# t-0hmura/pdb2reaction

Measured on AMD Instinct MI355X. Metric: path_opt_string_iterations_per_s, higher is better.
Workload: dtype bf16x3-split

## Files before the change

pdb2reaction_amd/csrc/gemm_bench.hip:

```cpp
#include <hip/hip_runtime.h>
#include <algorithm>
#include <cmath>
#include <cstdio>
#include <cstdlib>
#include <cstring>
#include <vector>
#include "umx_gemm_pl.h"
#include "umx_gemm_q.h"
using namespace umx;
#define CK(x) do { hipError_t e = (x); if (e != hipSuccess) { printf("HIP error %s at %s:%d\n", hipGetErrorString(e), __FILE__, __LINE__); exit(1); } } while (0)

template <class F> float timeit(F f, int reps = 5) {
  hipEvent_t a, b; CK(hipEventCreate(&a)); CK(hipEventCreate(&b));
  f(); CK(hipDeviceSynchronize());
  CK(hipEventRecord(a)); for (int i = 0; i < reps; ++i) f(); CK(hipEventRecord(b)); CK(hipEventSynchronize(b));
  float ms; CK(hipEventElapsedTime(&ms, a, b)); return ms / reps;
}

template <int P>
__global__ void k_split(const float* __restrict__ src, long rows, long ld, int K, unsigned short* __restrict__ dst) {
  const long i = (long)blockIdx.x * blockDim.x + threadIdx.x;
  if (i >= rows * K) return;
  const long r = i / K; const int k = (int)(i % K);
  float x = src[r * ld + k];
  for (int q = 0; q < P; ++q) { const __bf16 h = (__bf16)x; dst[r * K * P + (k / 32) * 32 * P + q * 32 + (k % 32)] = __builtin_bit_cast(unsigned short, h); x -= (float)h; }
}

template <int P>
__global__ void k_split_q(const float* __restrict__ src, long rows, long ld, int K, unsigned char* __restrict__ dst) {
  const long i = (long)blockIdx.x * blockDim.x + threadIdx.x;
  if (i >= rows * K) return;
  const long r = i / K; const int k = (int)(i % K);
  float x = src[r * ld + k];
  unsigned short* d = reinterpret_cast<unsigned short*>(dst + ((r / 4) * (K / 16) + k / 16) * (128 * P) + (r % 4) * (32 * P) + (k % 16) * 2);
  for (int q = 0; q < P; ++q) { const __bf16 hh = (__bf16)x; d[q * 16] = __builtin_bit_cast(unsigned short, hh); x -= (float)hh; }
}

template <int PQ>
__global__ void k_split_q_f16(const float* __restrict__ src, long rows, long ld, int K, unsigned char* __restrict__ dst) {
  const long i = (long)blockIdx.x * blockDim.x + threadIdx.x;
  if (i >= rows * K) return;
  const long r = i / K; const int k = (int)(i % K);
  float x = src[r * ld + k];
  unsigned short* d = reinterpret_cast<unsigned short*>(dst + ((r / 4) * (K / 16) + k / 16) * (128 * PQ) + (r % 4) * (32 * PQ) + (k % 16) * 2);
  for (int q = 0; q < PQ; ++q) { const _Float16 hq = (_Float16)x; d[16 * q] = __builtin_bit_cast(unsigned short, hq); x -= (float)hq; }
}

constexpr int Q8_SHIFT = 20;
constexpr int Q8_SHIFT1 = 10;
template <int WEIGHT>
__global__ void k_split_o8(const float* __restrict__ src, long rows, long ld, int K, unsigned char* __restrict__ dst) {
  const long i = (long)blockIdx.x * blockDim.x + threadIdx.x;
  if (i >= rows * K) return;
  const long r = i / K; const int k = (int)(i % K);
  const float x = src[r * ld + k];
  const _Float16 h0 = (_Float16)x; const _Float16 h1 = (_Float16)(x - (float)h0);
  const float r2 = (x - (float)h0) - (float)h1;
  const float xc = fminf(fmaxf(x, -57344.f), 57344.f), l1 = (float)h1 * (float)(1 << Q8_SHIFT1);
  const int pk = WEIGHT ? __builtin_amdgcn_cvt_pk_bf8_f32(xc, l1, 0, false) : __builtin_amdgcn_cvt_pk_bf8_f32(l1, r2 * (float)(1 << Q8_SHIFT), 0, false);
  unsigned char* d = dst + (r * (K / 64) + k / 64) * 128 + (k % 64);
  d[0] = (unsigned char)(pk & 0xff); d[64] = (unsigned char)((pk >> 8) & 0xff);
}


__global__ void k_copy_qf(const float* __restrict__ src, long rows, long ld, int K, unsigned char* __restrict__ dst) {
  const long i = (long)blockIdx.x * blockDim.x + threadIdx.x;
  if (i >= rows * K) return;
  const long r = i / K; const int k = (int)(i % K);
  *reinterpret_cast<float*>(dst + ((r / 4) * (K / 16) + k / 16) * 256 + (r % 4) * 64 + (k % 16) * 4) = src[r * ld + k];
}
typedef float f32x4_t __attribute__((ext_vector_type(4)));
typedef unsigned int u32x4_t __attribute__((ext_vector_type(4)));
#ifndef QF_TRUNC
#define QF_TRUNC 0
#endif
__device__ __forceinline__ void split3_pair(float x0, float x1, unsigned int& p0, unsigned int& p1, unsigned int& p2) {
#if QF_TRUNC
  const unsigned int u0 = __builtin_bit_cast(unsigned int, x0), u1 = __builtin_bit_cast(unsigned int, x1);
  p0 = __builtin_amdgcn_perm(u1, u0, 0x07060302u);
  const float r0 = x0 - __builtin_bit_cast(float, u0 & 0xffff0000u), r1 = x1 - __builtin_bit_cast(float, u1 & 0xffff0000u);
  const unsigned int v0 = __builtin_bit_cast(unsigned int, r0), v1 = __builtin_bit_cast(unsigned int, r1);
  p1 = __builtin_amdgcn_perm(v1, v0, 0x07060302u);
  const float s0 = r0 - __builtin_bit_cast(float, v0 & 0xffff0000u), s1 = r1 - __builtin_bit_cast(float, v1 & 0xffff0000u);
  p2 = __builtin_amdgcn_perm(__builtin_bit_cast(unsigned int, s1), __builtin_bit_cast(unsigned int, s0), 0x07060302u);
#else
  typedef float f32x2_t __attribute__((ext_vector_type(2)));
  typedef __bf16 bf16x2_t __attribute__((ext_vector_type(2)));
  p0 = __builtin_bit_cast(unsigned int, __builtin_convertvector(f32x2_t{x0, x1}, bf16x2_t));
  const float r0 = x0 - __builtin_bit_cast(float, p0 << 16), r1 = x1 - __builtin_bit_cast(float, p0 & 0xffff0000u);
  p1 = __builtin_bit_cast(unsigned int, __builtin_convertvector(f32x2_t{r0, r1}, bf16x2_t));
  const float s0 = r0 - __builtin_bit_cast(float, p1 << 16), s1 = r1 - __builtin_bit_cast(float, p1 & 0xffff0000u);
  p2 = __builtin_bit_cast(unsigned int, __builtin_convertvector(f32x2_t{s0, s1}, bf16x2_t));
#endif
}
template <int WIDE, int S>
__global__ __launch_bounds__(512, 1) void gemm_qf_kernel(const GemmPL p) {
  constexpr int PB = 3, BM = 256, BN = WIDE ? 256 : 128;
  constexpr int BLKB = 128 * PB, CPBB = 8 * PB;
  constexpr int A_BYTES = BM * 64, B_BYTES = BN * 32 * PB, STAGE = A_BYTES + B_BYTES;
  constexpr int TNW = WIDE ? 4 : 2;
  constexpr int JA = A_BYTES / 8192, JBF = B_BYTES / 8192, BHR = (B_BYTES % 8192) ? 1 : 0;
  static_assert(S * STAGE <= 160 * 1024, "LDS");
  __shared__ __attribute__((aligned(1024))) unsigned char ring[S * STAGE];
  const int tid = threadIdx.x, lane = tid & 63, wave = tid >> 6;
  const int wm = wave >> 1, wn = wave & 1;
  const int l31 = lane & 31, h = lane >> 5;
  const int nN = (p.N + BN - 1) / BN, nM = (p.M + BM - 1) / BM;
  const int xcd = blockIdx.x & 7, slot = blockIdx.x >> 3;
  const int mt = (slot / nN) * 8 + xcd, nt = slot % nN;
  if (mt >= nM) return;
  const unsigned char* Ab = reinterpret_cast<const unsigned char*>(p.Apl);
  const unsigned char* Bb = reinterpret_cast<const unsigned char*>(p.Bpl);
  const long a_blocks = p.lda / 16, b_blocks = p.K / 16;
  const long gA = ((long)p.M + 3) / 4;
  const int gN = p.N / 4;
  long a_off[JA], b_off[JBF + BHR];
#pragma unroll
  for (int j = 0; j < JA; ++j) {
    const int c = tid + 512 * j, g = c >> 4, s = c & 15;
    long grp = (long)mt * (BM / 4) + g;
    if (grp >= gA) grp = gA - 1;
    a_off[j] = grp * a_blocks * 256 + (s >> 2) * 64 + (((s & 3) ^ (g & 3)) * 16);
  }
#pragma unroll
  for (int j = 0; j < JBF + BHR; ++j) {
    const int c = tid + 512 * j, g = (c / CPBB) % (BN / 4), s = c % CPBB;
    int cg = nt * (BN / 4) + g; if (cg >= gN) cg = gN - 1;
    b_off[j] = (long)cg * b_blocks * BLKB + (s ^ q_swz<PB>(g)) * 16;
  }
  const int piece = __builtin_amdgcn_readfirstlane(wave * 1024);
  const bool b_tail = __builtin_amdgcn_readfirstlane(wave < 4 ? 1 : 0) != 0;
  f32x16 acc[2][TNW];
#pragma unroll
  for (int i = 0; i < 2; ++i)
#pragma unroll
    for (int j = 0; j < TNW; ++j)
#pragma unroll
      for (int r = 0; r < 16; ++r) acc[i][j][r] = 0.f;
  int a_ad[2][2], b_ad[TNW][PB];
#pragma unroll
  for (int t = 0; t < 2; ++t) {
    const int row = wm * 64 + t * 32 + l31, g = row >> 2;
#pragma unroll
    for (int i = 0; i < 2; ++i) a_ad[t][i] = g * 256 + (row & 3) * 64 + (((h * 2 + i) ^ (g & 3)) * 16);
  }
#pragma unroll
  for (int t = 0; t < TNW; ++t) {
    const int row = wn * (32 * TNW) + t * 32 + l31;
#pragma unroll
    for (int q = 0; q < PB; ++q) b_ad[t][q] = A_BYTES + q_row_off<PB>(row) + ((q * 2 + h) ^ q_swz<PB>(row >> 2)) * 16;
  }
  const int nk = p.K / 16;
  constexpr int GI = JA + JBF;
#pragma unroll
  for (int t = 0; t < S - 1; ++t)
    if (t < nk) q3_issue<JA, JBF, BHR, A_BYTES, kernel_tag<7, S, WIDE>()>(Ab, Bb, ring + t * STAGE, a_off, b_off, (long)t * 256, (long)t * BLKB, piece, b_tail);
  int st_cur = 0, st_nxt = S - 1;
  for (int kt = 0; kt < nk; ++kt) {
    if (S == 2 || kt + S - 2 >= nk) wait_vmcnt<0>();
    else if (BHR != 0 && b_tail) wait_vmcnt<(S - 2) * (GI + 1)>();
    else wait_vmcnt<(S - 2) * GI>();
    __builtin_amdgcn_s_barrier();
    if (kt + S - 1 < nk) q3_issue<JA, JBF, BHR, A_BYTES, kernel_tag<7, S, WIDE>()>(Ab, Bb, ring + st_nxt * STAGE, a_off, b_off, (long)(kt + S - 1) * 256, (long)(kt + S - 1) * BLKB, piece, b_tail);
    const unsigned char* sb = ring + st_cur * STAGE;
    st_cur = st_cur + 1 == S ? 0 : st_cur + 1;
    st_nxt = st_nxt + 1 == S ? 0 : st_nxt + 1;
    bf16x8_t a[2][3], b[TNW][PB];
#pragma unroll
    for (int t = 0; t < 2; ++t) {
      const f32x4_t lo = *reinterpret_cast<const f32x4_t*>(sb + a_ad[t][0]), hi = *reinterpret_cast<const f32x4_t*>(sb + a_ad[t][1]);
      unsigned int w[3][4];
      split3_pair(lo[0], lo[1], w[0][0], w[1][0], w[2][0]); split3_pair(lo[2], lo[3], w[0][1], w[1][1], w[2][1]);
      split3_pair(hi[0], hi[1], w[0][2], w[1][2], w[2][2]); split3_pair(hi[2], hi[3], w[0][3], w[1][3], w[2][3]);
#pragma unroll
      for (int q = 0; q < 3; ++q) { const u32x4_t v{w[q][0], w[q][1], w[q][2], w[q][3]}; a[t][q] = __builtin_bit_cast(bf16x8_t, v); }
    }
#pragma unroll
    for (int q = 0; q < PB; ++q)
#pragma unroll
      for (int t = 0; t < TNW; ++t) b[t][q] = *reinterpret_cast<const bf16x8_t*>(sb + b_ad[t][q]);
#pragma unroll
    for (int ord = 4; ord >= 0; --ord)
#pragma unroll
      for (int qa = 0; qa < 3; ++qa) {
        const int qb = ord - qa;
        if (qb < 0 || qb >= PB || qa + qb >= 3) continue;
#pragma unroll
        for (int i = 0; i < 2; ++i)
#pragma unroll
          for (int j = 0; j < TNW; ++j) acc[i][j] = __builtin_amdgcn_mfma_f32_32x32x16_bf16(a[i][qa], b[j][qb], acc[i][j], 0, 0, 0);
      }
  }
#pragma unroll
  for (int i = 0; i < 2; ++i)
#pragma unroll
    for (int j = 0; j < TNW; ++j) {
      const int col = nt * BN + wn * (32 * TNW) + j * 32 + l31;
      const long row0 = (long)mt * BM + wm * 64 + i * 32 + 4 * h;
      float* c = p.Cp + row0 * p.ldc + col;
      if (col < p.N)
#pragma unroll
        for (int r = 0; r < 16; ++r) {
          const int dr = (r & 3) + 8 * (r >> 2);
          if (row0 + dr < p.M) c[(long)dr * p.ldc] = acc[i][j][r];
        }
    }
}

static int f16_mode(long M, int N, int K) {
  float *A, *B, *C; unsigned char *Aq3, *Bq3, *Aq2, *Bq2;
  const long Mp = (M + 3) / 4 * 4;
  CK(hipMalloc(&A, M * (long)K * 4)); CK(hipMalloc(&B, (long)N * K * 4)); CK(hipMalloc(&C, M * (long)N * 4));
  CK(hipMalloc(&Aq3, (size_t)Mp * K * 6)); CK(hipMalloc(&Bq3, (size_t)N * K * 6)); CK(hipMalloc(&Aq2, (size_t)Mp * K * 4)); CK(hipMalloc(&Bq2, (size_t)N * K * 4));
  unsigned char* Bq3h; CK(hipMalloc(&Bq3h, (size_t)N * K * 6));
  unsigned char *A8, *B8; CK(hipMalloc(&A8, (size_t)Mp * K * 2)); CK(hipMalloc(&B8, (size_t)N * K * 2));
  const int R = 256;
  for (int ragged = 0; ragged < 2; ++ragged) {
    std::vector<float> h((size_t)1 << 22); for (auto& v : h) v = (rand() / (float)RAND_MAX) * 2 - 1;
    std::vector<float> ha((size_t)R * K), hb((size_t)N * K);
    for (int r = 0; r < R; ++r) for (int k = 0; k < K; ++k) ha[(size_t)r * K + k] = h[(size_t)r * K + k] * (ragged ? std::ldexp(1.f, -(r % 28)) : 1.f);
    for (size_t i = 0; i < hb.size(); ++i) hb[i] = 0.1f * h[(1 << 21) + i];
    for (long o = 0; o < M * (long)K; o += h.size()) CK(hipMemcpy(A + o, h.data(), std::min<long>(h.size(), M * (long)K - o) * 4, hipMemcpyHostToDevice));
    CK(hipMemcpy(A, ha.data(), ha.size() * 4, hipMemcpyHostToDevice));
    CK(hipMemcpy(B, hb.data(), hb.size() * 4, hipMemcpyHostToDevice));
    CK(hipMemset(Aq3, 0, (size_t)Mp * K * 6)); CK(hipMemset(Aq2, 0, (size_t)Mp * K * 4));
    hipLaunchKernelGGL(k_split_q<3>, dim3((unsigned)((M * K + 255) / 256)), dim3(256), 0, 0, A, M, (long)K, K, Aq3);
    hipLaunchKernelGGL(k_split_q<3>, dim3((unsigned)(((long)N * K + 255) / 256)), dim3(256), 0, 0, B, (long)N, (long)K, K, Bq3);
    hipLaunchKernelGGL(k_split_q_f16<2>, dim3((unsigned)((M * K + 255) / 256)), dim3(256), 0, 0, A, M, (long)K, K, Aq2);
    hipLaunchKernelGGL(k_split_q_f16<2>, dim3((unsigned)(((long)N * K + 255) / 256)), dim3(256), 0, 0, B, (long)N, (long)K, K, Bq2);
    hipLaunchKernelGGL(k_split_q_f16<3>, dim3((unsigned)(((long)N * K + 255) / 256)), dim3(256), 0, 0, B, (long)N, (long)K, K, Bq3h);
    CK(hipMemset(A8, 0, (size_t)Mp * K * 2));
    hipLaunchKernelGGL(k_split_o8<0>, dim3((unsigned)((M * K + 255) / 256)), dim3(256), 0, 0, A, M, (long)K, K, A8);
    hipLaunchKernelGGL(k_split_o8<1>, dim3((unsigned)(((long)N * K + 255) / 256)), dim3(256), 0, 0, B, (long)N, (long)K, K, B8);
    CK(hipDeviceSynchronize());
    std::vector<double> ref((size_t)R * N), nrm(R, 0.0);
    for (int r = 0; r < R; ++r) for (int n = 0; n < N; ++n) {
      double sacc = 0; for (int k = 0; k < K; ++k) sacc += (double)ha[(size_t)r * K + k] * (double)hb[(size_t)n * K + k];
      ref[(size_t)r * N + n] = sacc; nrm[r] = std::max(nrm[r], std::fabs(sacc));
    }
    GemmPL g3; std::memset(&g3, 0, sizeof(g3)); g3.conj = 1.f;
    g3.Apl = reinterpret_cast<const unsigned short*>(Aq3); g3.lda = 3L * K; g3.Bpl = reinterpret_cast<const unsigned short*>(Bq3); g3.ldb = 3L * K;
    g3.Cp = C; g3.ldc = N; g3.M = (int)M; g3.N = N; g3.K = K;
    g3.cscale = 1.f;
    GemmPL g2 = g3; g2.Apl = reinterpret_cast<const unsigned short*>(Aq2); g2.lda = 2L * K; g2.Bpl = reinterpret_cast<const unsigned short*>(Bq2); g2.ldb = 2L * K;
    GemmP pf; std::memset(&pf, 0, sizeof(pf)); pf.conj = 1.f; pf.A = A; pf.lda = K; pf.B = B; pf.ldb = K; pf.Cp = C; pf.ldc = N; pf.M = (int)M; pf.N = N; pf.K = K;
    const long nm = (M + 255) / 256; const dim3 gw((unsigned)(((nm + 7) / 8) * 8 * ((N + 255) / 256)));
    const long nM = (M + 127) / 128, nN = (N + 127) / 128; const dim3 gf((unsigned)(((nM + 7) / 8) * 8 * nN));
    const double fl = 2.0 * M * N * K;
    auto report = [&](const char* name, float ms) {
      std::vector<float> c((size_t)R * N); CK(hipMemcpy(c.data(), C, c.size() * 4, hipMemcpyDeviceToHost));
      double worst = 0, rms = 0, shrink = 0, wsum = 0;
      for (int r = 0; r < R; ++r) for (int n = 0; n < N; ++n) {
        const double rf = ref[(size_t)r * N + n], d = c[(size_t)r * N + n] - rf, e = std::fabs(d) / nrm[r];
        worst = std::max(worst, e); rms += e * e;
        shrink += d * rf / (nrm[r] * nrm[r]); wsum += rf * rf / (nrm[r] * nrm[r]);
      }
      printf("%s %-30s %8.3f ms %7.1f alg-TF/s   max rel err %.2e  rms %.2e  fitted gain-1 %+.2e\n", ragged ? "[ragged]" : "[flat]  ", name, ms, fl / ms / 1e9, worst, std::sqrt(rms / ((double)R * N)), shrink / wsum);
      fflush(stdout);
    };
    CK(hipMemset(C, 0, M * (long)N * 4));
    report("fp32 MFMA", timeit([&] { hipLaunchKernelGGL((umx_gemm_kernel<A_PLAIN, 0>), gf, dim3(256), 0, 0, pf); }));
    CK(hipMemset(C, 0, M * (long)N * 4));
    report("Q3 bf16 x3 planes, 6 products", timeit([&] { hipLaunchKernelGGL((umx_gemm_q_kernel<0, 1>), gw, dim3(512), 0, 0, g3); }));
    {
      unsigned char* Aqf; CK(hipMalloc(&Aqf, (size_t)Mp * K * 4)); CK(hipMemset(Aqf, 0, (size_t)Mp * K * 4));
      hipLaunchKernelGGL(k_copy_qf, dim3((unsigned)((M * K + 255) / 256)), dim3(256), 0, 0, A, M, (long)K, K, Aqf);
      CK(hipDeviceSynchronize());
      GemmPL gf = g3; gf.Apl = reinterpret_cast<const unsigned short*>(Aqf); gf.lda = K;
      CK(hipMemset(C, 0, M * (long)N * 4));
      report("A fp32 split in registers, 6 products", timeit([&] { hipLaunchKernelGGL((gemm_qf_kernel<1, 2>), gw, dim3(512), 0, 0, gf); }));
      {
        std::vector<float> c0((size_t)4096 * N), c1((size_t)4096 * N);
        auto cmp = [&](const char* nm) { CK(hipMemcpy(c1.data(), C, c1.size() * 4, hipMemcpyDeviceToHost)); size_t nd = 0; for (size_t i = 0; i < c0.size(); ++i) nd += std::memcmp(&c0[i], &c1[i], 4) != 0; printf("         %-44s differing from the plane form in %zu of %zu values\n", nm, nd, c0.size()); };
        CK(hipMemset(C, 0, M * (long)N * 4)); hipLaunchKernelGGL((umx_gemm_q_kernel<0, 1>), gw, dim3(512), 0, 0, g3); CK(hipDeviceSynchronize());
        CK(hipMemcpy(c0.data(), C, c0.size() * 4, hipMemcpyDeviceToHost));
        CK(hipMemset(C, 0, M * (long)N * 4)); hipLaunchKernelGGL((gemm_qf_kernel<1, 2>), gw, dim3(512), 0, 0, gf); CK(hipDeviceSynchronize()); cmp("bench kernel gemm_qf_kernel<1, 2>");
        CK(hipMemset(C, 0, M * (long)N * 4)); GemmPL gl = gf; gl.lda = 3L * K;
        hipLaunchKernelGGL((umx_gemm_q_kernel<0, 1, 3, 2, 0, 6, 3, 1>), gw, dim3(512), 0, 0, gl); CK(hipDeviceSynchronize()); cmp("library kernel AF = 1, 256x256");
        const dim3 gn2((unsigned)(((nm + 7) / 8) * 8 * ((N + 127) / 128)));
        CK(hipMemset(C, 0, M * (long)N * 4)); hipLaunchKernelGGL((umx_gemm_q_kernel<0, 0, 3, 2, 0, 6, 3, 1>), gn2, dim3(512), 0, 0, gl); CK(hipDeviceSynchronize()); cmp("library kernel AF = 1, 256x128");
        CK(hipMemset(C, 0, M * (long)N * 4)); hipLaunchKernelGGL((umx_gemm_q_kernel<0, 0>), gn2, dim3(512), 0, 0, g3); CK(hipDeviceSynchronize()); cmp("library kernel planes, 256x128");
      }
      CK(hipMemset(C, 0, M * (long)N * 4));
      report("... ring 3", timeit([&] { hipLaunchKernelGGL((gemm_qf_kernel<1, 3>), gw, dim3(512), 0, 0, gf); }));
      const dim3 gn((unsigned)(((nm + 7) / 8) * 8 * ((N + 127) / 128)));
      CK(hipMemset(C, 0, M * (long)N * 4));
      report("... 256x128 tiles", timeit([&] { hipLaunchKernelGGL((gemm_qf_kernel<0, 2>), gn, dim3(512), 0, 0, gf); }));
      CK(hipMemset(C, 0, M * (long)N * 4));
      report("Q3 bf16 x3, 256x128 tiles", timeit([&] { hipLaunchKernelGGL((umx_gemm_q_kernel<0, 0>), gn, dim3(512), 0, 0, g3); }));
      CK(hipFree(Aqf));
    }
    CK(hipMemset(C, 0, M * (long)N * 4));
    report("Q2 f16 x2 planes, 4 products", timeit([&] { hipLaunchKernelGGL((umx_gemm_q_kernel<0, 1, 2, 2, 1, 4, 2>), gw, dim3(512), 0, 0, g2); }));
    CK(hipMemset(C, 0, M * (long)N * 4));
    report("Q2 f16 x2 planes, 3 products", timeit([&] { hipLaunchKernelGGL((umx_gemm_q_kernel<0, 1, 2, 2, 1, 3, 2>), gw, dim3(512), 0, 0, g2); }));
    CK(hipMemset(C, 0, M * (long)N * 4));
    { GemmPL g23 = g2; g23.Bpl = reinterpret_cast<const unsigned short*>(Bq3h); g23.ldb = 3L * K; g23.cscale = 1.f;
      CK(hipMemset(C, 0, M * (long)N * 4));
      report("f16 A x2 / B x3 exact, 4 products", timeit([&] { hipLaunchKernelGGL((umx_gemm_q_kernel<0, 1, 2, 2, 1, 4, 3>), gw, dim3(512), 0, 0, g23); }));
      CK(hipMemset(C, 0, M * (long)N * 4));
      report("f16 A x2 / B x3, 5 products", timeit([&] { hipLaunchKernelGGL((umx_gemm_q_kernel<0, 1, 2, 2, 1, 5, 3>), gw, dim3(512), 0, 0, g23); })); }
    CK(hipMemset(C, 0, M * (long)N * 4));
    report("Q2 f16 x2, 4 products, ring 3", timeit([&] { hipLaunchKernelGGL((umx_gemm_q_kernel<0, 1, 2, 3, 1, 4, 2>), gw, dim3(512), 0, 0, g2); }));
  }
  return 0;
}

__global__ void k_count_diff(const unsigned int* __restrict__ a, const unsigned int* __restrict__ b, long n, unsigned long long* __restrict__ out) {
  unsigned long long d = 0;
  for (long i = (long)blockIdx.x * blockDim.x + threadIdx.x; i < n; i += (long)gridDim.x * blockDim.x) d += a[i] != b[i];
  if (d) atomicAdd(out, d);
}
static int half_mode(long M) {
  struct Shape { const char* name; int cplx, wide, N, K, a_cols, offA1, bHalf, ldc, offCi; void (*full)(const GemmPL); void (*half)(const GemmPL); };
  const Shape shapes[] = {
      {"conv-1 m0  plain 256x128 LS=2", 0, 0, 640, 768, 768, 0, 0, 640, 0, umx_gemm_q_kernel<0, 0, 3, 2, 0, 6, 3, 1, 2, 1>, umx_gemm_q_kernel<0, 0, 3, 2, 0, 6, 3, 1, 2, 1, 2>},
      {"conv-2 m0  plain 256x128 LS=2", 0, 0, 384, 384, 384, 0, 0, 384, 0, umx_gemm_q_kernel<0, 0, 3, 2, 0, 6, 3, 1, 2, 1>, umx_gemm_q_kernel<0, 0, 3, 2, 0, 6, 3, 1, 2, 1, 2>},
      {"fc3        plain 256x256 LS=1", 0, 1, 1536, 128, 128, 0, 0, 1536, 0, umx_gemm_q_kernel<0, 1, 3, 2, 0, 6, 3, 1, 1, 1>, umx_gemm_q_kernel<0, 1, 3, 2, 0, 6, 3, 1, 1, 1, 2>},
      {"conv m>0   complex 256x256", 1, 1, 256, 512, 1024, 512, 256, 512, 256, umx_gemm_q_kernel<1, 1, 3, 2, 0, 6, 3, 1>, umx_gemm_q_kernel<1, 1, 3, 2, 0, 6, 3, 1, 0, 0, 2>},
  };
  const long Mp = (M + 3) / 4 * 4;
  std::vector<float> h((size_t)1 << 22); for (auto& v : h) v = (rand() / (float)RAND_MAX) * 2 - 1;
  unsigned long long* d_nd; CK(hipMalloc(&d_nd, 8));
  for (const Shape& sh : shapes) {
    const int brows = sh.cplx ? 2 * sh.bHalf : sh.N;
    float *A, *B, *C0, *C1, *bias; unsigned char *Aqf, *Bq;
    const size_t an = (size_t)M * sh.a_cols, bn = (size_t)brows * sh.K, cn = (size_t)M * sh.ldc;
    CK(hipMalloc(&A, an * 4)); CK(hipMalloc(&B, bn * 4)); CK(hipMalloc(&C0, cn * 4)); CK(hipMalloc(&C1, cn * 4)); CK(hipMalloc(&bias, sh.N * 4));
    CK(hipMalloc(&Aqf, (size_t)Mp * sh.a_cols * 4)); CK(hipMalloc(&Bq, bn * 6));
    for (size_t o = 0; o < an; o += h.size() - 977) CK(hipMemcpy(A + o, h.data() + (o % 977), std::min(h.size() - 977, an - o) * 4, hipMemcpyHostToDevice));
    CK(hipMemcpy(B, h.data() + 13, bn * 4, hipMemcpyHostToDevice)); CK(hipMemcpy(bias, h.data() + 5, sh.N * 4, hipMemcpyHostToDevice));
    CK(hipMemset(Aqf, 0, (size_t)Mp * sh.a_cols * 4));
    hipLaunchKernelGGL(k_copy_qf, dim3((unsigned)((an + 255) / 256)), dim3(256), 0, 0, A, M, (long)sh.a_cols, sh.a_cols, Aqf);
    hipLaunchKernelGGL(k_split_q<3>, dim3((unsigned)((bn + 255) / 256)), dim3(256), 0, 0, B, (long)brows, (long)sh.K, sh.K, Bq);
    CK(hipDeviceSynchronize());
    GemmPL g; std::memset(&g, 0, sizeof(g)); g.conj = 1.f; g.cscale = 1.f; g.odd_sign = -1.f;
    g.Apl = reinterpret_cast<const unsigned short*>(Aqf); g.lda = 3L * sh.a_cols; g.offA0 = 0; g.offA1 = sh.offA1;
    g.Bpl = reinterpret_cast<const unsigned short*>(Bq); g.ldb = 3L * sh.K; g.bHalf = sh.bHalf; g.bias = sh.cplx ? nullptr : bias;
    g.ldc = sh.ldc; g.offC = 0; g.offCi = sh.offCi; g.M = (int)M; g.N = sh.N; g.K = sh.K;
    const int bnc = (sh.wide ? 256 : 128) / (sh.cplx ? 2 : 1), nN = (sh.N + bnc - 1) / bnc;
    auto grid = [&](int bm) { const int bmr = sh.cplx ? bm / 2 : bm; const long nM = (M + bmr - 1) / bmr; return dim3((unsigned)(((nM + 7) / 8) * 8 * nN)); };
    GemmPL g0 = g, g1 = g; g0.Cp = C0; g1.Cp = C1;
    CK(hipMemset(C0, 0, cn * 4)); CK(hipMemset(C1, 0xff, cn * 4));
    const float t0 = timeit([&] { hipLaunchKernelGGL(sh.full, grid(256), dim3(512), 0, 0, g0); });
    const float t1 = timeit([&] { hipLaunchKernelGGL(sh.half, grid(128), dim3(256), 0, 0, g1); });
    const float t0b = timeit([&] { hipLaunchKernelGGL(sh.full, grid(256), dim3(512), 0, 0, g0); });
    const float t1b = timeit([&] { hipLaunchKernelGGL(sh.half, grid(128), dim3(256), 0, 0, g1); });
    CK(hipMemset(d_nd, 0, 8));
    hipLaunchKernelGGL(k_count_diff, dim3(4096), dim3(256), 0, 0, reinterpret_cast<const unsigned int*>(C0), reinterpret_cast<const unsigned int*>(C1), (long)cn, d_nd);
    unsigned long long nd = 0; CK(hipMemcpy(&nd, d_nd, 8, hipMemcpyDeviceToHost));
    const double fl = (sh.cplx ? 8.0 : 2.0) * M * sh.N * sh.K * 6;
    printf("%-32s M %ld N %4d K %4d   256-row %7.3f / %7.3f ms (%6.0f TF/s executed)   128-row x2 %7.3f / %7.3f ms (%6.0f TF/s)   %+5.1f %%   differing output words %llu of %zu\n",
           sh.name, M, sh.N, sh.K, t0, t0b, fl / std::min(t0, t0b) / 1e9, t1, t1b, fl / std::min(t1, t1b) / 1e9, 100.0 * (std::min(t1, t1b) / std::min(t0, t0b) - 1.0), nd, cn);
    fflush(stdout);
    CK(hipFree(A)); CK(hipFree(B)); CK(hipFree(C0)); CK(hipFree(C1)); CK(hipFree(bias)); CK(hipFree(Aqf)); CK(hipFree(Bq));
  }
  return 0;
}

int main(int argc, char** argv) {
  if (argc > 1 && !strcmp(argv[1], "half")) return half_mode(argc > 2 ? atol(argv[2]) : 1140000);
  if (argc > 1 && !strcmp(argv[1], "f16")) return f16_mode(argc > 2 ? atol(argv[2]) : 569632, argc > 3 ? atoi(argv[3]) : 512, argc > 4 ? atoi(argv[4]) : 512);
  const long M = argc > 1 ? atol(argv[1]) : 569632; const int N = argc > 2 ? atoi(argv[2]) : 640, K = argc > 3 ? atoi(argv[3]) : 768;
  const long lda = 2304;
  float *A, *C, *C2, *B; unsigned short *Bp, *Ap, *Bp2, *Ap2;
  CK(hipMalloc(&A, M * lda * 4)); CK(hipMalloc(&C, M * (long)N * 4)); CK(hipMalloc(&C2, M * (long)N * 4)); CK(hipMalloc(&B, (long)N * K * 4));
  CK(hipMalloc(&Bp, 3L * N * K * 2)); CK(hipMalloc(&Ap, 3L * M * K * 2)); CK(hipMalloc(&Bp2, 2L * N * K * 2)); CK(hipMalloc(&Ap2, 2L * M * K * 2));
  std::vector<float> h(1 << 22); for (auto& v : h) v = (rand() / (float)RAND_MAX) * 2 - 1;
  for (long o = 0; o < M * lda; o += h.size()) CK(hipMemcpy(A + o, h.data() + (o % 977), std::min<long>(h.size() - 977, M * lda - o) * 4, hipMemcpyHostToDevice));
  CK(hipMemcpy(B, h.data() + 13, (long)N * K * 4, hipMemcpyHostToDevice));
  hipLaunchKernelGGL(k_split<3>, dim3((unsigned)((M * K + 255) / 256)), dim3(256), 0, 0, A, M, lda, K, Ap);
  hipLaunchKernelGGL(k_split<3>, dim3((unsigned)(((long)N * K + 255) / 256)), dim3(256), 0, 0, B, (long)N, (long)K, K, Bp);
  hipLaunchKernelGGL(k_split<2>, dim3((unsigned)((M * K + 255) / 256)), dim3(256), 0, 0, A, M, lda, K, Ap2);
  hipLaunchKernelGGL(k_split<2>, dim3((unsigned)(((long)N * K + 255) / 256)), dim3(256), 0, 0, B, (long)N, (long)K, K, Bp2);
  CK(hipDeviceSynchronize());
  GemmP p; std::memset(&p, 0, sizeof(p)); p.conj = 1.f;
  p.A = A; p.lda = lda; p.B = B; p.ldb = K; p.Cp = C; p.ldc = N; p.M = (int)M; p.N = N; p.K = K;
  GemmPL q; std::memset(&q, 0, sizeof(q)); q.conj = 1.f;
  q.Apl = Ap; q.lda = 3L * K; q.Bpl = Bp; q.ldb = 3L * K; q.Cp = C2; q.ldc = N; q.M = (int)M; q.N = N; q.K = K;
  GemmPL q2 = q; q2.Apl = Ap2; q2.lda = 2L * K; q2.Bpl = Bp2; q2.ldb = 2L * K;
  const long nM = (M + 127) / 128, nN = (N + 127) / 128; dim3 grid((unsigned)(((nM + 7) / 8) * 8 * nN)), block(256);
  const double fl = 2.0 * M * N * K;
  auto rep = [&](const char* name, float ms) { printf("%-44s %8.3f ms  %7.1f alg-TFLOP/s\n", name, ms, fl / ms / 1e9); fflush(stdout); };
  auto check = [&](const char* name) {
    const long rows = std::min<long>(M, 300);
    std::vector<float> c1(rows * N), c2(rows * N), c3(200L * N), c4(200L * N);
    CK(hipMemcpy(c1.data(), C, rows * N * 4, hipMemcpyDeviceToHost)); CK(hipMemcpy(c2.data(), C2, rows * N * 4, hipMemcpyDeviceToHost));
    CK(hipMemcpy(c3.data(), C + (M - 200) * N, 200L * N * 4, hipMemcpyDeviceToHost)); CK(hipMemcpy(c4.data(), C2 + (M - 200) * N, 200L * N * 4, hipMemcpyDeviceToHost));
    double md = 0, mr = 0;
    for (size_t i = 0; i < c1.size(); ++i) { md = std::max(md, (double)std::fabs(c1[i] - c2[i])); mr = std::max(mr, (double)std::fabs(c1[i])); }
    for (size_t i = 0; i < c3.size(); ++i) md = std::max(md, (double)std::fabs(c3[i] - c4[i]));
    printf("   check %-30s max|diff| %.3e (max|ref| %.3e)\n", name, md, mr);
    if (getenv("DBG")) { for (int r : {0, 1, 33, 130}) { printf("     row %d ref:", r); for (int c : {0, 1, 31, 32, 64, 100}) printf(" %9.4f", c1[(size_t)r * N + c]); printf("\n     row %d got:", r); for (int c : {0, 1, 31, 32, 64, 100}) printf(" %9.4f", c2[(size_t)r * N + c]); printf("\n"); } }
  };
  rep("fp32 PLAIN", timeit([&] { hipLaunchKernelGGL((umx_gemm_kernel<A_PLAIN, 0>), grid, block, 0, 0, p); }));
  auto launch_pl = [&](void (*k)(const GemmPL), dim3 g, const GemmPL& a, int nthr = 256) { hipLaunchKernelGGL(k, g, dim3(nthr), 0, 0, a); };
  auto gridpl = [&](int bn) { const long nm = (M + 255) / 256, nn = (N + bn - 1) / bn; return dim3((unsigned)(((nm + 7) / 8) * 8 * nn)); };
  CK(hipMemset(C2, 0, M * (long)N * 4));
  rep("PL 8w 256x128 P=3 S=2", timeit([&] { launch_pl(&umx_gemm_pl_kernel<32, 0, 3, 2, 4, 2, 2, 2>, gridpl(128), q, 512); }));
  check("PL 8w 256x128 P=3 S=2 vs fp32");
  CK(hipMemset(C2, 0, M * (long)N * 4));
  rep("PL 8w 256x128 P=2 S=3", timeit([&] { launch_pl(&umx_gemm_pl_kernel<32, 0, 2, 3, 4, 2, 2, 2>, gridpl(128), q2, 512); }));
  check("PL 8w 256x128 P=2 S=3 vs fp32");
  CK(hipMemset(C2, 0, M * (long)N * 4));
  rep("PL16 8w 256x128 P=3 S=2 (16x16x32)", timeit([&] { launch_pl(&umx_gemm_pl_kernel<16, 0, 3, 2, 4, 2, 2, 2>, gridpl(128), q, 512); }));
  check("PL16 P=3 vs fp32");
  CK(hipMemset(C2, 0, M * (long)N * 4));
  rep("PL16 8w 256x128 P=2 S=3 (16x16x32)", timeit([&] { launch_pl(&umx_gemm_pl_kernel<16, 0, 2, 3, 4, 2, 2, 2>, gridpl(128), q2, 512); }));
  check("PL16 P=2 vs fp32");
  {
    auto grid128 = [&](int bn) { const long nm = (M + 127) / 128, nn = (N + bn - 1) / bn; return dim3((unsigned)(((nm + 7) / 8) * 8 * nn)); };
    CK(hipMemset(C2, 0, M * (long)N * 4));
    rep("PL16 4w 128x128 P=2 S=2 (2 blocks/CU)", timeit([&] { launch_pl(&umx_gemm_pl_kernel<16, 0, 2, 2, 2, 2, 2, 2>, grid128(128), q2, 256); }));
    check("PL16 4w 128x128 P=2 vs fp32");
    CK(hipMemset(C2, 0, M * (long)N * 4));
    rep("PL32 4w 128x128 P=2 S=2 (2 blocks/CU)", timeit([&] { launch_pl(&umx_gemm_pl_kernel<32, 0, 2, 2, 2, 2, 2, 2>, grid128(128), q2, 256); }));
    check("PL32 4w 128x128 P=2 vs fp32");
  }
  if (N % 256 == 0) {
    unsigned char *Aq2, *Bq2;
    const long Mp2 = (M + 3) / 4 * 4;
    CK(hipMalloc(&Aq2, (size_t)Mp2 * K * 4)); CK(hipMalloc(&Bq2, (size_t)N * K * 4));
    CK(hipMemset(Aq2, 0, (size_t)Mp2 * K * 4));
    hipLaunchKernelGGL(k_split_q<2>, dim3((unsigned)((M * K + 255) / 256)), dim3(256), 0, 0, A, M, lda, K, Aq2);
    hipLaunchKernelGGL(k_split_q<2>, dim3((unsigned)(((long)N * K + 255) / 256)), dim3(256), 0, 0, B, (long)N, (long)K, K, Bq2);
    CK(hipDeviceSynchronize());
    GemmPL g2; std::memset(&g2, 0, sizeof(g2)); g2.conj = 1.f;
    g2.Apl = reinterpret_cast<const unsigned short*>(Aq2); g2.lda = 2L * K; g2.Bpl = reinterpret_cast<const unsigned short*>(Bq2); g2.ldb = 2L * K;
    g2.Cp = C2; g2.ldc = N; g2.M = (int)M; g2.N = N; g2.K = K;
    CK(hipMemset(C2, 0, M * (long)N * 4));
    rep("Q2 256x256 P=2 (quad-row, BK=16)", timeit([&] { hipLaunchKernelGGL((umx_gemm_q_kernel<0, 1, 2>), gridpl(256), dim3(512), 0, 0, g2); }));
    check("Q2 256x256 P=2 vs fp32");
    CK(hipMemset(C2, 0, M * (long)N * 4));
    rep("Q2 256x128 P=2 (quad-row, BK=16)", timeit([&] { hipLaunchKernelGGL((umx_gemm_q_kernel<0, 0, 2>), gridpl(128), dim3(512), 0, 0, g2); }));
    check("Q2 256x128 P=2 vs fp32");
    CK(hipFree(Aq2)); CK(hipFree(Bq2));
  }
  if (N % 256 == 0) {
    unsigned char *Aq, *Bq;
    const long Mp = (M + 3) / 4 * 4;
    CK(hipMalloc(&Aq, (size_t)Mp * K * 6)); CK(hipMalloc(&Bq, (size_t)N * K * 6));
    CK(hipMemset(Aq, 0, (size_t)Mp * K * 6));
    hipLaunchKernelGGL(k_split_q<3>, dim3((unsigned)((M * K + 255) / 256)), dim3(256), 0, 0, A, M, lda, K, Aq);
    hipLaunchKernelGGL(k_split_q<3>, dim3((unsigned)(((long)N * K + 255) / 256)), dim3(256), 0, 0, B, (long)N, (long)K, K, Bq);
    CK(hipDeviceSynchronize());
    GemmPL gq; std::memset(&gq, 0, sizeof(gq)); gq.conj = 1.f;
    gq.Apl = reinterpret_cast<const unsigned short*>(Aq); gq.lda = 3L * K; gq.Bpl = reinterpret_cast<const unsigned short*>(Bq); gq.ldb = 3L * K;
    gq.Cp = C2; gq.ldc = N; gq.M = (int)M; gq.N = N; gq.K = K;
    CK(hipMemset(C2, 0, M * (long)N * 4));
    rep("Q3 256x256 P=3 (quad-row layout, BK=16)", timeit([&] { hipLaunchKernelGGL((umx_gemm_q_kernel<0, 1>), gridpl(256), dim3(512), 0, 0, gq); }));
    check("Q3 256x256 P=3 vs fp32");
    CK(hipMemset(C2, 0, M * (long)N * 4));
    rep("Q3 256x128 P=3", timeit([&] { hipLaunchKernelGGL((umx_gemm_q_kernel<0, 0>), gridpl(128), dim3(512), 0, 0, gq); }));
    check("Q3 256x128 P=3 vs fp32");
    CK(hipFree(Aq)); CK(hipFree(Bq));
  }
  if (N % 256 == 0) {
    CK(hipMemset(C2, 0, M * (long)N * 4));
    rep("PL32 8w 256x256 P=2 S=2 (wave 128x64)", timeit([&] { launch_pl(&umx_gemm_pl_kernel<32, 0, 2, 2, 2, 4, 4, 2>, gridpl(256), q2, 512); }));
    check("PL32 256x256 P=2 vs fp32");
    CK(hipMemset(C2, 0, M * (long)N * 4));
    rep("PL16 8w 256x256 P=2 S=2 (wave 128x64)", timeit([&] { launch_pl(&umx_gemm_pl_kernel<16, 0, 2, 2, 2, 4, 4, 2>, gridpl(256), q2, 512); }));
    check("PL16 256x256 P=2 vs fp32");
    CK(hipMemset(C2, 0, M * (long)N * 4));
    rep("PL16 8w 256x256 P=2 S=2 (wave 64x128)", timeit([&] { launch_pl(&umx_gemm_pl_kernel<16, 0, 2, 2, 4, 2, 2, 4>, gridpl(256), q2, 512); }));
    check("PL16 256x256 b P=2 vs fp32");
  }
  return 0;
}
```

pdb2reaction_amd/csrc/umx_api.hip:

```cpp
#include "umx_engine.h"
#include "umx_launch.h"
#include "umx_workspace.h"
#include "umx_periodic.h"
#include "umx_virial.h"
#include "umx_plan.h"
#include "umx_weights.h"
#include "umx_experts.h"

#define NOT_MERGED "expert-form weights are loaded but not merged: call umx_set_expert_coefficients first (then umx_set_system)"

namespace {
int energy_forces_dev_impl(umx_engine* eng, int n_images, const PosPtr d_pos, double* d_energy, float* d_forces, double* d_virial, void* hip_stream) {
  if (!eng) return UMX_ERR_ARG;
  if (eng->need_merge()) return fail(eng, UMX_ERR_ARG, "umx_energy_forces: " NOT_MERGED);
  if (!eng->have_system) return fail(eng, UMX_ERR_ARG, "umx_energy_forces: bind a system first (umx_set_system)");
  if (n_images <= 0 || !(d_pos.f || d_pos.d) || !d_energy) return fail(eng, UMX_ERR_ARG, "umx_energy_forces: bad arguments");
  if (d_virial && !d_forces) return fail(eng, UMX_ERR_ARG, "umx_energy_forces_virial: the virial comes out of the reverse pass: ask for the forces too");
  if (eng->gp_plan) return fail(eng, UMX_ERR_ARG, "umx_energy_forces: a graph-parallel evaluation is in progress (finish it with umx_gp_step)");
  CHK(periodic_check_images(eng, n_images, "umx_energy_forces"));
  HIPCHK(eng, hipSetDevice(eng->dev));
  return energy_forces_on(eng, static_cast<hipStream_t>(hip_stream), n_images, d_pos, d_energy, d_forces, d_virial);
}

template <typename P>
int energy_forces_host_impl(umx_engine* eng, int n_images, const P* pos, double* energy, float* forces, double* virial) {
  if (!eng) return UMX_ERR_ARG;
  if (eng->need_merge()) return fail(eng, UMX_ERR_ARG, "umx_energy_forces: " NOT_MERGED);
  if (!eng->have_system) return fail(eng, UMX_ERR_ARG, "umx_energy_forces: bind a system first (umx_set_system)");
  if (n_images <= 0 || !pos || !energy) return fail(eng, UMX_ERR_ARG, "umx_energy_forces: bad arguments");
  if (virial && !forces) return fail(eng, UMX_ERR_ARG, "umx_energy_forces_virial: the virial comes out of the reverse pass: ask for the forces too");
  if (eng->gp_plan) return fail(eng, UMX_ERR_ARG, "umx_energy_forces: a graph-parallel evaluation is in progress (finish it with umx_gp_step)");
  CHK(periodic_check_images(eng, n_images, "umx_energy_forces"));
  HIPCHK(eng, hipSetDevice(eng->dev));
  const long nt = (long)n_images * eng->natoms;
  if (eng->io_cap < nt) CHK(grow(eng, eng->io_cap, nt, {eng->stream}, {DevBuf(eng->d_io_pos, nt * 3), DevBuf(eng->d_io_f, nt * 3)}));
  if (eng->io_img_cap < n_images) CHK(grow(eng, eng->io_img_cap, (long)n_images, {eng->stream}, {DevBuf(eng->d_io_e, n_images)}));
  if (virial && eng->io_w_cap < n_images) CHK(grow(eng, eng->io_w_cap, (long)n_images, {eng->stream}, {DevBuf(eng->d_io_w, (size_t)n_images * 9)}));
  P* d_stage;
  if constexpr (std::is_same_v<P, double>) {
    if (eng->io64_cap < nt) CHK(grow(eng, eng->io64_cap, nt, {eng->stream}, {DevBuf(eng->d_io_pos64, nt * 3)}));
    d_stage = eng->d_io_pos64;
  } else d_stage = eng->d_io_pos;
  for (long i = 0; i < nt * 3; ++i)
    if (!std::isfinite(pos[i])) return fail(eng, UMX_ERR_ARG, "umx_energy_forces: non-finite position (image " + std::to_string(i / ((long)eng->natoms * 3)) + ")");
  HIPCHK(eng, hipMemcpyAsync(d_stage, pos, nt * 3 * sizeof(P), hipMemcpyHostToDevice, eng->stream));
  CHK(energy_forces_on(eng, eng->stream, n_images, PosPtr(d_stage), eng->d_io_e, forces ? eng->d_io_f : nullptr, virial ? eng->d_io_w : nullptr));
  HIPCHK(eng, hipMemcpyAsync(energy, eng->d_io_e, (size_t)n_images * sizeof(double), hipMemcpyDeviceToHost, eng->stream));
  if (forces) HIPCHK(eng, hipMemcpyAsync(forces, eng->d_io_f, nt * 3 * sizeof(float), hipMemcpyDeviceToHost, eng->stream));
  if (virial) HIPCHK(eng, hipMemcpyAsync(virial, eng->d_io_w, (size_t)n_images * 9 * sizeof(double), hipMemcpyDeviceToHost, eng->stream));
  HIPCHK(eng, hipStreamSynchronize(eng->stream));
  for (int k = 0; k < n_images; ++k)
    if (!std::isfinite(energy[k])) {
      (void)hipMemset(eng->d_flags, 0, sizeof(int));
      return fail(eng, UMX_ERR_RANGE, "image " + std::to_string(k) + ": non-finite energy" +
                  (eng->prec.fwd_f16() ? " (an activation beyond the fp16 operand range of UMX_PRECISION=split: try split-bf16, bf16x3 or fp32)"
                                      : " (an overflow in float32)"));
    }
  return UMX_OK;
}

void pin_clear(umx_engine* eng) { eng->pin_on = false; }

int pin_after_cell(umx_engine* eng) {
  if (!eng->pin_on) return UMX_OK;
  bool same = eng->pbc_on == eng->pin_pbc_on;
  for (int k = 0; k < 3 && same && eng->pbc_on; ++k) same = eng->pbc[k] == eng->pin_pbc[k];
  if (!same) { pin_clear(eng); return UMX_OK; }
  const int st = pin_upload_shifts(eng, eng->pin_codes, &eng->d_pin_shifts, &eng->pin_shifts_cap);
  if (st != UMX_OK) pin_clear(eng);
  return st;
}

template <typename P>
int pin_graph_impl(umx_engine* eng, const P* pos) {
  if (!eng) return UMX_ERR_ARG;
  if (eng->need_merge()) return fail(eng, UMX_ERR_ARG, "umx_pin_graph: " NOT_MERGED);
  if (!eng->have_system) return fail(eng, UMX_ERR_ARG, "umx_pin_graph: bind a system first (umx_set_system)");
  if (!pos) return fail(eng, UMX_ERR_ARG, "umx_pin_graph: bad arguments");
  if (eng->gp_plan) return fail(eng, UMX_ERR_ARG, "umx_pin_graph: a graph-parallel evaluation is in progress (finish it with umx_gp_step)");
  CHK(periodic_check_images(eng, 1, "umx_pin_graph"));
  const int N = eng->natoms;
  for (long i = 0; i < (long)N * 3; ++i)
    if (!std::isfinite(pos[i])) return fail(eng, UMX_ERR_ARG, "umx_pin_graph: non-finite position");
  HIPCHK(eng, hipSetDevice(eng->dev));
  hipStream_t s = eng->stream;
  HIPCHK(eng, hipStreamSynchronize(s));
  if (eng->ran_on_caller) HIPCHK(eng, hipEventSynchronize(eng->ev_done));
  if (eng->io_cap < N) CHK(grow(eng, eng->io_cap, (long)N, {s}, {DevBuf(eng->d_io_pos, (size_t)N * 3), DevBuf(eng->d_io_f, (size_t)N * 3)}));
  P* d_stage;
  if constexpr (std::is_same_v<P, double>) {
    if (eng->io64_cap < N) CHK(grow(eng, eng->io64_cap, (long)N, {s}, {DevBuf(eng->d_io_pos64, (size_t)N * 3)}));
    d_stage = eng->d_io_pos64;
  } else d_stage = eng->d_io_pos;
  HIPCHK(eng, hipMemcpyAsync(d_stage, pos, (size_t)N * 3 * sizeof(P), hipMemcpyHostToDevice, s));
  struct Keep {
    umx_engine* e; bool pin; int64_t edges; int32_t maxdeg; int shifts; bool trunc;
    ~Keep() { e->pin_on = pin; e->last_edges = edges; e->last_maxdeg = maxdeg; e->last_shifts = shifts; e->may_truncate = trunc; }
  } keep{eng, eng->pin_on, eng->last_edges, eng->last_maxdeg, eng->last_shifts, eng->may_truncate};
  eng->pin_on = false;
  PosPtr dp(d_stage);
  CHK(periodic_prepare(eng, s, 1, &dp));
  ImageEdges ie;
  CHK(degree_pass(eng, s, 1, dp, ie));
  const long E = ie.etot;
  const bool trunc = eng->may_truncate;
  int *n_src = nullptr, *n_dst = nullptr, *n_tix = nullptr, *n_wrap = nullptr, *t_row = nullptr;
  float* t_evec = nullptr;
  float4* n_shifts = nullptr; long n_shifts_cap = 0;
  struct Bufs { void** p[7]; bool drop = true; ~Bufs() { if (drop) for (void** q : p) if (*q) (void)hipFree(*q); } }
      bufs{{(void**)&n_src, (void**)&n_dst, (void**)&n_tix, (void**)&n_wrap, (void**)&t_row, (void**)&t_evec, (void**)&n_shifts}};
  const size_t eb = (size_t)std::max(E, 1L);
  HIPCHK(eng, hipMalloc(&n_src, eb * sizeof(int)));
  HIPCHK(eng, hipMalloc(&n_dst, eb * sizeof(int)));
  HIPCHK(eng, hipMalloc(&n_tix, eb * sizeof(int)));
  HIPCHK(eng, hipMalloc(&n_wrap, (size_t)N * 3 * sizeof(int)));
  HIPCHK(eng, hipMalloc(&t_row, ((size_t)N + 3) * sizeof(int)));
  HIPCHK(eng, hipMalloc(&t_evec, eb * 4 * sizeof(float)));
  HIPCHK(eng, hipMemsetAsync(n_tix, 0, eb * sizeof(int), s));
  HIPCHK(eng, hipMemsetAsync(n_wrap, 0, (size_t)N * 3 * sizeof(int), s));
  hipLaunchKernelGGL(k_scan, dim3(1), dim3(1024), 0, s, eng->d_deg_all, (long)N, t_row, t_row + N + 1);
  launch_graph_fill_pin(eng, s, trunc, dp, (long)N, eng->d_cand_all, t_row, n_src, n_dst, t_evec, n_tix);
  if (eng->pbc_on) launch_wrap_index_of(eng, s, d_stage, n_wrap);
  HIPCHK(eng, hipGetLastError());
  std::vector<int> deg((size_t)N), code(eb);
  HIPCHK(eng, hipMemcpyAsync(deg.data(), eng->d_deg_all, (size_t)N * sizeof(int), hipMemcpyDeviceToHost, s));
  if (E > 0) HIPCHK(eng, hipMemcpyAsync(code.data(), n_tix, (size_t)E * sizeof(int), hipMemcpyDeviceToHost, s));
  HIPCHK(eng, hipStreamSynchronize(s));
  std::vector<long> row((size_t)N + 1, 0);
  int maxdeg = 0;
  for (int i = 0; i < N; ++i) { row[i + 1] = row[i] + deg[i]; maxdeg = std::max(maxdeg, deg[i]); }
  if (row[N] != E) return fail(eng, UMX_ERR_HIP, "umx_pin_graph: the degrees and the edge count of the reference graph disagree");
  std::vector<unsigned> codes;
  if (eng->pbc_on && E > 0) {
    const std::set<unsigned> uniq(code.begin(), code.begin() + E);
    codes.assign(uniq.begin(), uniq.end());
    for (long e = 0; e < E; ++e) code[e] = (int)(std::lower_bound(codes.begin(), codes.end(), (unsigned)code[e]) - codes.begin());
    HIPCHK(eng, hipMemcpy(n_tix, code.data(), (size_t)E * sizeof(int), hipMemcpyHostToDevice));
  }
  CHK(pin_upload_shifts(eng, codes, &n_shifts, &n_shifts_cap));
  bufs.drop = false;
  void* old[] = {eng->d_pin_src, eng->d_pin_dst, eng->d_pin_tix, eng->d_pin_wrap, eng->d_pin_shifts, eng->d_pin_deg, t_row, t_evec};
  for (void* q : old) if (q) (void)hipFree(q);
  eng->d_pin_src = n_src; eng->d_pin_dst = n_dst; eng->d_pin_tix = n_tix; eng->d_pin_wrap = n_wrap;
  eng->d_pin_shifts = n_shifts; eng->pin_shifts_cap = n_shifts_cap;
  eng->d_pin_deg = nullptr; eng->pin_deg_imgs = 0;
  eng->pin_deg = std::move(deg); eng->pin_row = std::move(row); eng->pin_codes = std::move(codes);
  eng->pin_edges = E; eng->pin_maxdeg = maxdeg;
  eng->pin_pbc_on = eng->pbc_on;
  for (int k = 0; k < 3; ++k) eng->pin_pbc[k] = eng->pbc_on ? eng->pbc[k] : 0;
  keep.pin = true;
  return UMX_OK;
}
}

extern "C" {

int umx_abi_version(void) { return 10; }

#ifndef UMX_SRC_DIGEST
#define UMX_SRC_DIGEST "unknown"
#endif
const char* umx_build_digest(void) { return UMX_SRC_DIGEST; }

const char* umx_last_error(const umx_engine* eng) { return eng ? eng->err.c_str() : g_create_err.c_str(); }

int umx_create(umx_engine** out, int device_ordinal) {
  if (!out) { g_create_err = "umx_create: null out pointer"; return UMX_ERR_ARG; }
  *out = nullptr;
  int n = 0;
  if (hipGetDeviceCount(&n) != hipSuccess || n <= 0) { g_create_err = "umx_create: no HIP device visible"; return UMX_ERR_NO_DEVICE; }
  if (device_ordinal < 0 || device_ordinal >= n) { g_create_err = "umx_create: device ordinal out of range"; return UMX_ERR_ARG; }
  hipDeviceProp_t prop;
  if (hipGetDeviceProperties(&prop, device_ordinal) != hipSuccess) { g_create_err = "umx_create: hipGetDeviceProperties failed"; return UMX_ERR_HIP; }
  if (std::string(prop.gcnArchName).rfind("gfx950", 0) != 0) {
    g_create_err = std::string("umx_create: device is ") + prop.gcnArchName + ", this library is built for gfx950 only";
    return UMX_ERR_NO_DEVICE;
  }
  umx_engine* e = new umx_engine();
  e->dev = device_ordinal;
  if (const char* ev = std::getenv("UMX_STREAMS")) e->n_lanes = std::atoi(ev) >= 2 ? 2 : (std::atoi(ev) == 1 ? 1 : 0);
  if (const char* ev = std::getenv("UMX_LANES_AUTO_EDGES")) e->lanes_auto_edges = std::max(0L, std::atol(ev));
  if (const char* ev = std::getenv("UMX_FORCE_PARTS")) e->force_parts = std::max(0, std::min(16, std::atoi(ev)));
  if (const char* ev = std::getenv("UMX_RECOMPUTE")) e->recompute = std::max(0, std::min(2, std::atoi(ev)));
  if (const char* ev = std::getenv("UMX_WS_GB")) e->ws_cap_default = (size_t)std::max(0L, std::atol(ev)) << 30;
  if (const char* ev = std::getenv("UMX_WS_EAGER")) e->ws_eager = std::atoi(ev) != 0;
  if (const char* ev = std::getenv("UMX_WS_SOFT_EDGES")) e->ws_soft_edges = std::max(1L, std::atol(ev));
  if (const char* ev = std::getenv("UMX_NODE_F64")) e->node_f64_on = std::atoi(ev) != 0;
  if (const char* ev = std::getenv("UMX_GRID_F64")) e->grid_f64 = std::atoi(ev) != 0;
  if (const char* ev = std::getenv("UMX_ALT_ROWS")) e->odd_sign = std::atoi(ev) != 0 ? -1.0f : 1.0f;
  if (const char* ev = std::getenv("UMX_LOW_SEP")) e->low_sep = std::atoi(ev);
  if (const char* ev = std::getenv("UMX_GEMM_HALF")) e->gemm_half = std::atoi(ev);
  if (const char* ev = std::getenv("UMX_ALIGN_PLANES")) e->align = std::atoi(ev);
  int prio_lo = 0, prio_hi = 0;
  if (hipSetDevice(device_ordinal) != hipSuccess || hipDeviceGetStreamPriorityRange(&prio_lo, &prio_hi) != hipSuccess ||
      hipStreamCreateWithFlags(&e->stream, hipStreamNonBlocking) != hipSuccess ||
      hipStreamCreateWithPriority(&e->stream2, hipStreamNonBlocking, prio_hi) != hipSuccess ||
      hipEventCreateWithFlags(&e->ev_fork, hipEventDisableTiming) != hipSuccess || hipEventCreateWithFlags(&e->ev_join, hipEventDisableTiming) != hipSuccess ||
      hipEventCreateWithFlags(&e->ev_tok[0], hipEventDisableTiming) != hipSuccess || hipEventCreateWithFlags(&e->ev_tok[1], hipEventDisableTiming) != hipSuccess ||
      hipEventCreateWithFlags(&e->ev_done, hipEventDisableTiming) != hipSuccess || hipMalloc(&e->d_flags, 4 * sizeof(int)) != hipSuccess ||
      hipMemset(e->d_flags, 0, 4 * sizeof(int)) != hipSuccess) {
    g_create_err = "umx_create: hipSetDevice/hipStreamCreate failed";
    delete e;
    return UMX_ERR_HIP;
  }
  *out = e;
  return UMX_OK;
}


int umx_destroy(umx_engine* eng) {
  if (!eng) return UMX_OK;
  gp_clear(eng);
  (void)hipSetDevice(eng->dev);
  (void)hipStreamSynchronize(eng->stream);
  for (auto& r : eng->prof) { (void)hipEventDestroy(r.a); (void)hipEventDestroy(r.b); }
  void* ptrs[] = {eng->d_w, eng->d_dw, eng->d_bw, eng->d_gmu, eng->d_z, eng->d_sysemb, eng->arena, eng->d_deg_all, eng->d_cand_all, eng->d_img_edges, eng->d_io_pos, eng->d_io_e, eng->d_io_f, eng->d_flags, eng->d_dtab, eng->d_part_deg, eng->d_part_f, eng->d_ex, eng->d_mjobs, eng->d_pjobs, eng->d_mx, eng->d_shifts, eng->d_cells, eng->d_shifts_pk, eng->d_wrap, eng->d_wrap64, eng->d_lats, eng->d_io_pos64, eng->d_vir_part, eng->d_vir_wp, eng->d_io_w, eng->d_pin_src, eng->d_pin_dst, eng->d_pin_tix, eng->d_pin_wrap, eng->d_pin_deg, eng->d_pin_shifts};
  for (void* p : ptrs) if (p) (void)hipFree(p);
  (void)hipStreamSynchronize(eng->stream2);
  (void)hipEventDestroy(eng->ev_fork); (void)hipEventDestroy(eng->ev_join);
  (void)hipEventDestroy(eng->ev_tok[0]); (void)hipEventDestroy(eng->ev_tok[1]);
  if (eng->ev_done) (void)hipEventDestroy(eng->ev_done);
  if (eng->ev_m0) { (void)hipEventDestroy(eng->ev_m0); (void)hipEventDestroy(eng->ev_m1); }
  (void)hipStreamDestroy(eng->stream2);
  (void)hipStreamDestroy(eng->stream);
  delete eng;
  return UMX_OK;
}

int umx_set_workspace_limit(umx_engine* eng, size_t bytes) {
  if (!eng) return UMX_ERR_ARG;
  eng->ws_limit = bytes;
  return UMX_OK;
}

int umx_load_weights(umx_engine* eng, const void* blob, size_t nbytes) {
  if (!eng || !blob) return UMX_ERR_ARG;
  return load_weights_impl(eng, blob, nbytes);
}

int umx_set_expert_coefficients(umx_engine* eng, int n, const double* alpha) {
  if (!eng) return UMX_ERR_ARG;
  return set_expert_coefficients_impl(eng, n, alpha);
}

int umx_expert_count(const umx_engine* eng) { return eng && eng->have_weights ? eng->n_experts : 0; }

const char* umx_precision_mode(const umx_engine* eng) {
  if (!eng || !eng->have_weights) return "";
  return eng->prec.name;
}

const char* umx_model_variant(const umx_engine* eng) {
  if (!eng || !eng->have_weights) return "";
  return eng->variant.c_str();
}

int umx_set_system(umx_engine* eng, int n_atoms, const int32_t* z, int charge, int spin, int task_index, float radius, int max_neigh) {
  if (!eng) return UMX_ERR_ARG;
  if (!eng->have_weights) return fail(eng, UMX_ERR_ARG, "umx_set_system: load weights first");
  if (eng->need_merge()) return fail(eng, UMX_ERR_ARG, "umx_set_system: " NOT_MERGED);
  if (n_atoms <= 0 || !z) return fail(eng, UMX_ERR_ARG, "umx_set_system: empty system");
  if (charge < -100 || charge > 100) return fail(eng, UMX_ERR_ARG, "umx_set_system: charge outside [-100, 100]");
  if (spin < 0 || spin > 100) return fail(eng, UMX_ERR_ARG, "umx_set_system: spin multiplicity outside [0, 100]");
  if (eng->n_datasets > 0 && (task_index < 0 || task_index >= eng->n_datasets))
    return fail(eng, UMX_ERR_ARG, "umx_set_system: task index outside [0, " + std::to_string(eng->n_datasets - 1) + "] (rows of the blob's dataset_embedding.weight)");
  HIPCHK(eng, hipSetDevice(eng->dev));
  double rs = 0.0;
  for (int i = 0; i < n_atoms; ++i) {
    if (z[i] < 0 || z[i] >= NZ) return fail(eng, UMX_ERR_ARG, "umx_set_system: atomic number outside [0, 99]");
    rs += eng->elem_refs[z[i]];
  }
  HIPCHK(eng, hipStreamSynchronize(eng->stream));
  pin_clear(eng);
  if (eng->d_z) { HIPCHK(eng, hipFree(eng->d_z)); eng->d_z = nullptr; }
  HIPCHK(eng, hipMalloc(&eng->d_z, n_atoms * sizeof(int)));
  HIPCHK(eng, hipMemcpy(eng->d_z, z, n_atoms * sizeof(int), hipMemcpyHostToDevice));
  if (!eng->d_sysemb) HIPCHK(eng, hipMalloc(&eng->d_sysemb, C * sizeof(double)));
  {
    const float* hw = eng->h_w.data();
    auto HW = [&](const std::string& nm) -> const float* { return hw + eng->wt[nm].off; };
    double chg[C], spn[C], dst[C];
    auto emb = [&](const char* which, int v, bool is_spin, double* out) {
      const std::string pre = std::string(which) + "_embedding.";
      if (eng->emb_type == 1) {
        const float* w = HW(pre + "W");
        for (int k = 0; k < C / 2; ++k) {
          const double ang = 2.0 * 3.14159265358979323846 * (double)v * (double)w[k];
          out[k] = (is_spin && v == 0) ? 0.0 : std::sin(ang);
          out[C / 2 + k] = (is_spin && v == 0) ? 0.0 : std::cos(ang);
        }
      } else if (eng->emb_type == 2) {
        const float *w = HW(pre + "lin_emb.weight"), *b = HW(pre + "lin_emb.bias");
        const double x = (is_spin && v == 0) ? -100.0 : (double)v;
        for (int k = 0; k < C; ++k) out[k] = (double)w[k] * x + (double)b[k];
      } else {
        const float* t = HW(pre + "weight") + (size_t)(v + (is_spin ? 0 : 100)) * C;
        for (int k = 0; k < C; ++k) out[k] = t[k];
      }
    };
    emb("charge", charge, false, chg);
    emb("spin", spin, true, spn);
    const int nd = eng->n_datasets;
    for (int k = 0; k < C; ++k) dst[k] = nd ? (double)HW("dataset_embedding.weight")[(size_t)task_index * C + k] : 0.0;
    const float* mw = HW("mix_csd.weight");
    const float* mb = HW("mix_csd.bias");
    const size_t ldm = (size_t)(nd ? 3 : 2) * C;
    double se[C];
    for (int o = 0; o < C; ++o) {
      double acc = mb[o];
      for (int k = 0; k < C; ++k) {
        if (nd) acc += (double)mw[o * ldm + k] * chg[k] + (double)mw[o * ldm + C + k] * spn[k] + (double)mw[o * ldm + 2 * C + k] * dst[k];
        else acc += (double)mw[o * ldm + k] * chg[k] + (double)mw[o * ldm + C + k] * spn[k];
      }
      se[o] = acc / (1.0 + std::exp(-acc));
    }
    HIPCHK(eng, hipMemcpy(eng->d_sysemb, se, sizeof(se), hipMemcpyHostToDevice));
  }
  eng->natoms = n_atoms;
  eng->refsum = rs;
  eng->cutoff = radius > 0.f ? radius : 6.0f;
  {
    const double delta = (double)eng->cutoff / (NG - 1);
    double mu[NG];
    for (int k = 0; k < NG; ++k) mu[k] = k * delta;
    eng->gcoef = -0.5 / ((2.0 * delta) * (2.0 * delta));
    if (!eng->d_gmu) HIPCHK(eng, hipMalloc(&eng->d_gmu, NG * sizeof(double)));
    HIPCHK(eng, hipMemcpy(eng->d_gmu, mu, sizeof(mu), hipMemcpyHostToDevice));
  }
  eng->max_neigh = max_neigh > 0 ? max_neigh : 300;
  eng->have_system = true;
  return UMX_OK;
}

int umx_synchronize(umx_engine* eng) {
  if (!eng) return UMX_ERR_ARG;
  HIPCHK(eng, hipSetDevice(eng->dev));
  HIPCHK(eng, hipStreamSynchronize(eng->stream));
  if (eng->ran_on_caller) HIPCHK(eng, hipEventSynchronize(eng->ev_done));
  int flag = 0;
  HIPCHK(eng, hipMemcpy(&flag, eng->d_flags, sizeof(int), hipMemcpyDeviceToHost));
  if (flag) {
    HIPCHK(eng, hipMemset(eng->d_flags, 0, sizeof(int)));
    return fail(eng, UMX_ERR_RANGE, std::string("a device-pointer evaluation produced a non-finite energy") +
                ((flag & 2) ? " (a non-finite position reached an evaluation on the pinned graph)" : eng->prec.range_hint()));
  }
  return UMX_OK;
}

int umx_energy_forces_dev(umx_engine* eng, int n_images, const float* d_pos, double* d_energy, float* d_forces, void* hip_stream) {
  return umx_energy_forces_virial_dev(eng, n_images, d_pos, d_energy, d_forces, nullptr, hip_stream);
}

int umx_energy_forces_virial_dev(umx_engine* eng, int n_images, const float* d_pos, double* d_energy, float* d_forces, double* d_virial, void* hip_stream) {
  return energy_forces_dev_impl(eng, n_images, PosPtr(d_pos), d_energy, d_forces, d_virial, hip_stream);
}

int umx_energy_forces_f64_dev(umx_engine* eng, int n_images, const double* d_pos, double* d_energy, float* d_forces, double* d_virial, void* hip_stream) {
  return energy_forces_dev_impl(eng, n_images, PosPtr(d_pos), d_energy, d_forces, d_virial, hip_stream);
}

int umx_gp_begin(umx_engine* eng, const float* d_pos, int node_lo, int node_hi, double* d_energy, float* d_forces, void* hip_stream) {
  return umx_gp_begin_virial(eng, d_pos, node_lo, node_hi, d_energy, d_forces, nullptr, hip_stream);
}

int umx_gp_begin_virial(umx_engine* eng, const float* d_pos, int node_lo, int node_hi, double* d_energy, float* d_forces, double* d_virial, void* hip_stream) {
  if (!eng) return UMX_ERR_ARG;
  if (eng->need_merge()) return fail(eng, UMX_ERR_ARG, "umx_gp_begin: " NOT_MERGED);
  if (!eng->have_system) return fail(eng, UMX_ERR_ARG, "umx_gp_begin: bind a system first (umx_set_system)");
  if (!d_pos || !d_energy || !d_forces) return fail(eng, UMX_ERR_ARG, "umx_gp_begin: bad arguments (forces are part of the exchange)");
  if (node_lo < 0 || node_hi > eng->natoms || node_lo > node_hi) return fail(eng, UMX_ERR_ARG, "umx_gp_begin: node range outside [0, n_atoms]");
  if (eng->recompute == 2)
    return fail(eng, UMX_ERR_ARG, "umx_gp_begin: recompute mode 2 (umx_set_recompute / UMX_RECOMPUTE=2) is a one-GPU plan; the multi-GPU graph-parallel mode "
                                  "keeps every rank's activations stored: set mode 0 or 1 on the engines that take part");
  if (eng->pin_on)
    return fail(eng, UMX_ERR_ARG, "umx_gp_begin: a graph is pinned (umx_pin_graph) and the graph-parallel entries build their own: call umx_unpin_graph first");
  if (eng->pbc_on && eng->n_cells > 1)
    return fail(eng, UMX_ERR_ARG, "umx_gp_begin: one image, but umx_set_cells bound cells for " + std::to_string(eng->n_cells) +
                                  " images: the graph-parallel mode takes per-image cells only when exactly one is bound");
  if (eng->gp_plan) gp_clear(eng);
  HIPCHK(eng, hipSetDevice(eng->dev));
  eng->gp = true; eng->gp_lo = node_lo; eng->gp_hi = node_hi;
  const int st = energy_forces_on(eng, static_cast<hipStream_t>(hip_stream), 1, d_pos, d_energy, d_forces, d_virial);
  if (st != UMX_OK) gp_clear(eng);
  return st;
}

int umx_gp_step(umx_engine* eng, float** d_buf, size_t* count, int* done) {
  if (!eng || !d_buf || !count || !done) return UMX_ERR_ARG;
  if (!eng->gp_plan) return fail(eng, UMX_ERR_ARG, "umx_gp_step: no graph-parallel evaluation in progress (umx_gp_begin)");
  HIPCHK(eng, hipSetDevice(eng->dev));
  hipStream_t own = eng->stream;
  eng->stream = eng->gp_stream;
  *d_buf = nullptr; *count = 0; *done = 0;
  const Seg* stop = nullptr;
  int st = eng->gp_plan->run_to_sync(eng->gp_at, &stop);
  eng->stream = own;
  if (stop) { *d_buf = stop->sync_buf; *count = stop->sync_count; return UMX_OK; }
  if (st == UMX_OK) {
    *done = 1;
    eng->ran_on_caller = true;
    hipError_t e = hipEventRecord(eng->ev_done, eng->gp_stream);
    if (e != hipSuccess) st = fail(eng, UMX_ERR_HIP, std::string("umx_gp_step: ") + hipGetErrorName(e));
  }
  gp_clear(eng);
  return st;
}

namespace {
struct PeerState {
  hipEvent_t ev_in[PEER_MAX] = {}, ev_out[PEER_MAX] = {};
  int ev_dev[PEER_MAX];
  std::set<std::pair<int, int>> enabled;
  PeerState() { for (int& d : ev_dev) d = -1; }
} g_peer;

int peer_fail(int code, const std::string& msg) { g_create_err = msg; return code; }

#define PEERCHK(expr)                                                                                          \
  do {                                                                                                         \
    hipError_t _e = (expr);                                                                                    \
    if (_e != hipSuccess) { (void)hipSetDevice(dev0); return peer_fail(UMX_ERR_HIP, std::string("umx_peer_sum: " #expr ": ") + hipGetErrorName(_e)); } \
  } while (0)
}

int umx_peer_sum(int n_peers, float* const* d_bufs, size_t count, const int* device_ordinals, void* const* hip_streams) {
  if (n_peers < 1 || n_peers > PEER_MAX || !d_bufs || !device_ordinals || !hip_streams)
    return peer_fail(UMX_ERR_ARG, "umx_peer_sum: 1.." + std::to_string(PEER_MAX) + " participants with buffers, device ordinals and streams");
  int ndev = 0, dev0 = 0;
  if (hipGetDeviceCount(&ndev) != hipSuccess || ndev <= 0 || hipGetDevice(&dev0) != hipSuccess) return peer_fail(UMX_ERR_NO_DEVICE, "umx_peer_sum: no HIP device visible");
  PeerBufs b{};
  for (int r = 0; r < n_peers; ++r) {
    if (!d_bufs[r] || (reinterpret_cast<uintptr_t>(d_bufs[r]) & 15) != 0) return peer_fail(UMX_ERR_ARG, "umx_peer_sum: buffer " + std::to_string(r) + " is null or not 16-byte aligned");
    if (device_ordinals[r] < 0 || device_ordinals[r] >= ndev) return peer_fail(UMX_ERR_ARG, "umx_peer_sum: device ordinal of participant " + std::to_string(r) + " out of range");
    for (int q = 0; q < r; ++q)
      if (d_bufs[q] == d_bufs[r]) return peer_fail(UMX_ERR_ARG, "umx_peer_sum: participants " + std::to_string(q) + " and " + std::to_string(r) + " list the same buffer");
    b.p[r] = d_bufs[r];
  }
  if (n_peers == 1 || count == 0) return UMX_OK;
  for (int r = 0; r < n_peers; ++r)
    for (int q = 0; q < n_peers; ++q) {
      const int a = device_ordinals[r], c = device_ordinals[q];
      if (a == c || g_peer.enabled.count({a, c})) continue;
      int can = 0;
      PEERCHK(hipDeviceCanAccessPeer(&can, a, c));
      if (!can) return peer_fail(UMX_ERR_HIP, "umx_peer_sum: device " + std::to_string(a) + " cannot access the memory of device " + std::to_string(c) +
                                 " (hipDeviceCanAccessPeer = 0): the in-process pool needs peer access between all of its devices");
      PEERCHK(hipSetDevice(a));
      const hipError_t e = hipDeviceEnablePeerAccess(c, 0);
      if (e != hipSuccess && e != hipErrorPeerAccessAlreadyEnabled) {
        (void)hipSetDevice(dev0);
        return peer_fail(UMX_ERR_HIP, "umx_peer_sum: peer access from device " + std::to_string(a) + " to device " + std::to_string(c) + " cannot be enabled: " + hipGetErrorName(e));
      }
      (void)hipGetLastError();
      g_peer.enabled.insert({a, c});
    }
  for (int r = 0; r < n_peers; ++r) {
    if (g_peer.ev_dev[r] == device_ordinals[r]) continue;
    if (g_peer.ev_dev[r] >= 0) { PEERCHK(hipSetDevice(g_peer.ev_dev[r])); (void)hipEventDestroy(g_peer.ev_in[r]); (void)hipEventDestroy(g_peer.ev_out[r]); g_peer.ev_dev[r] = -1; }
    PEERCHK(hipSetDevice(device_ordinals[r]));
    PEERCHK(hipEventCreateWithFlags(&g_peer.ev_in[r], hipEventDisableTiming));
    PEERCHK(hipEventCreateWithFlags(&g_peer.ev_out[r], hipEventDisableTiming));
    g_peer.ev_dev[r] = device_ordinals[r];
  }
  for (int r = 0; r < n_peers; ++r) {
    PEERCHK(hipSetDevice(device_ordinals[r]));
    PEERCHK(hipEventRecord(g_peer.ev_in[r], static_cast<hipStream_t>(hip_streams[r])));
  }
  for (int r = 0; r < n_peers; ++r) {
    hipStream_t s = static_cast<hipStream_t>(hip_streams[r]);
    PEERCHK(hipSetDevice(device_ordinals[r]));
    for (int q = 0; q < n_peers; ++q)
      if (q != r) PEERCHK(hipStreamWaitEvent(s, g_peer.ev_in[q], 0));
    size_t lo, hi;
    peer_slice(count, n_peers, r, &lo, &hi);
    PEERCHK(launch_peer_sum(b, n_peers, lo, hi, s));
    PEERCHK(hipEventRecord(g_peer.ev_out[r], s));
  }
  for (int r = 0; r < n_peers; ++r) {
    PEERCHK(hipSetDevice(device_ordinals[r]));
    for (int q = 0; q < n_peers; ++q)
      if (q != r) PEERCHK(hipStreamWaitEvent(static_cast<hipStream_t>(hip_streams[r]), g_peer.ev_out[q], 0));
  }
  (void)hipSetDevice(dev0);
  return UMX_OK;
}

int umx_energy_forces(umx_engine* eng, int n_images, const float* pos, double* energy, float* forces) {
  return umx_energy_forces_virial(eng, n_images, pos, energy, forces, nullptr);
}

int umx_energy_forces_virial(umx_engine* eng, int n_images, const float* pos, double* energy, float* forces, double* virial) {
  return energy_forces_host_impl(eng, n_images, pos, energy, forces, virial);
}

int umx_energy_forces_f64(umx_engine* eng, int n_images, const double* pos, double* energy, float* forces, double* virial) {
  return energy_forces_host_impl(eng, n_images, pos, energy, forces, virial);
}

int umx_set_precision(umx_engine* eng, const char* mode) {
  if (!eng) return UMX_ERR_ARG;
  const std::string m = mode ? mode : "";
  if (!m.empty() && !resolve_precision(m, nullptr))
    return fail(eng, UMX_ERR_ARG, "umx_set_precision: mode must be auto, split, split-f16, split-bf16, bf16x3 (= split-exact) or fp32");
  eng->precision = m;
  return UMX_OK;
}

int umx_last_graph_stats(const umx_engine* eng, int64_t* n_edges_total, int32_t* max_degree) {
  if (!eng) return UMX_ERR_ARG;
  if (n_edges_total) *n_edges_total = eng->last_edges;
  if (max_degree) *max_degree = eng->last_maxdeg;
  return UMX_OK;
}

int umx_set_cell(umx_engine* eng, const double cell[9], const int pbc[3]) {
  if (!eng) return UMX_ERR_ARG;
  if (eng->gp_plan) return fail(eng, UMX_ERR_ARG, "umx_set_cell: a graph-parallel evaluation is in progress (finish it with umx_gp_step)");
  CHK(set_cell_impl(eng, cell, pbc));
  return pin_after_cell(eng);
}
int umx_set_cells(umx_engine* eng, int n_images, const double* cells, const int pbc[3]) {
  if (!eng) return UMX_ERR_ARG;
  if (eng->gp_plan) return fail(eng, UMX_ERR_ARG, "umx_set_cells: a graph-parallel evaluation is in progress (finish it with umx_gp_step)");
  CHK(set_cells_impl(eng, n_images, cells, pbc));
  return pin_after_cell(eng);
}
int umx_last_graph_shifts(const umx_engine* eng) { return eng ? eng->last_shifts : 0; }

int umx_pin_graph(umx_engine* eng, const float* pos_ang) { return pin_graph_impl(eng, pos_ang); }
int umx_pin_graph_f64(umx_engine* eng, const double* pos_ang) { return pin_graph_impl(eng, pos_ang); }
int umx_unpin_graph(umx_engine* eng) {
  if (!eng) return UMX_ERR_ARG;
  pin_clear(eng);
  return UMX_OK;
}
int umx_pinned_graph(const umx_engine* eng, int64_t* n_edges, int32_t* max_degree) {
  if (!eng) return UMX_ERR_ARG;
  if (n_edges) *n_edges = eng->pin_on ? (int64_t)eng->pin_edges : 0;
  if (max_degree) *max_degree = eng->pin_on ? (int32_t)eng->pin_maxdeg : 0;
  return UMX_OK;
}

int umx_last_partitions(const umx_engine* eng) { return eng ? eng->last_parts : 0; }
int umx_last_lanes(const umx_engine* eng) { return eng ? eng->last_lanes : 0; }

int umx_set_recompute(umx_engine* eng, int mode) {
  if (!eng) return UMX_ERR_ARG;
  if (mode < 0 || mode > 2) return fail(eng, UMX_ERR_ARG, "umx_set_recompute: mode must be 0 (off), 1 (when the stored plans do not fit) or 2 (always)");
  if (eng->gp_plan) return fail(eng, UMX_ERR_ARG, "umx_set_recompute: a graph-parallel evaluation is in progress (finish it with umx_gp_step)");
  eng->recompute = mode;
  return UMX_OK;
}
int umx_last_recompute(const umx_engine* eng) { return eng ? eng->last_recompute : 0; }

int64_t umx_workspace_bytes(const umx_engine* eng, int64_t n_nodes, int64_t n_edges, int parts, int recompute) {
  if (n_nodes < 0 || n_edges < 0 || parts < 0 || parts == 1 || parts > 16) return -1;
  const Precision pm = eng && eng->have_weights ? eng->prec : Precision();
  const int grid = eng && eng->have_weights ? eng->ws_grid() : 0;
  if (parts == 0) return (int64_t)carve(nullptr, n_nodes, n_edges, nullptr, pm, grid, recompute != 0);
  std::vector<long> pe(parts);
  for (int p = 0; p < parts; ++p) pe[p] = (long)(n_edges * (p + 1) / parts - n_edges * p / parts);
  return (int64_t)part_layout(pm, grid, recompute != 0, n_nodes, pe, nullptr);
}

int umx_workspace_stats(const umx_engine* eng, int64_t* bytes, int32_t* allocations) {
  if (!eng) return UMX_ERR_ARG;
  if (bytes) *bytes = (int64_t)eng->arena_bytes;
  if (allocations) *allocations = eng->arena_allocs;
  return UMX_OK;
}

int umx_reserve_images(umx_engine* eng, int n_images) {
  if (!eng) return UMX_ERR_ARG;
  if (n_images < 0) return fail(eng, UMX_ERR_ARG, "umx_reserve_images: n_images must be >= 0");
  eng->hint_images = n_images;
  if (n_images == 0) eng->hint_applied = 0;
  return UMX_OK;
}

int umx_profile_enable(umx_engine* eng, int on) {
  if (!eng) return UMX_ERR_ARG;
  eng->prof_on = on != 0;
  return UMX_OK;
}

int umx_profile_read(umx_engine* eng, umx_profile_stats* out, int reset) {
  if (!eng) return UMX_ERR_ARG;
  if (out) std::memset(out, 0, sizeof(*out));
  HIPCHK(eng, hipSetDevice(eng->dev));
  HIPCHK(eng, hipStreamSynchronize(eng->stream));
  if (eng->prof_used) HIPCHK(eng, hipEventSynchronize(eng->prof[eng->prof_used - 1].b));
  FILE* dump = nullptr;
  if (const char* dp = std::getenv("UMX_PROFILE_DUMP")) dump = std::fopen(dp, "a");
  for (size_t i = 0; i < eng->prof_used; ++i) {
    float t = 0.f;
    HIPCHK(eng, hipEventElapsedTime(&t, eng->prof[i].a, eng->prof[i].b));
    const ProfRec& r = eng->prof[i];
    if (out) {
      const int fam = r.prec > 0 ? 0 : (r.prec < 0 ? 2 : 1);
      out->ms[fam] += t; out->launches[fam] += 1; out->alg_flops[fam] += r.flops;
      out->mfma_flops[fam] += r.flops * (r.prec == 3 ? 6.0 : r.prec == 2 ? 3.0 : r.prec == 24 ? 4.0 : r.prec == 23 ? 3.0 : r.prec == 28 ? 6.0 : 1.0);
    }
    if (dump) std::fprintf(dump, "%d,%d,%d,%d,%d,%d,%d,%.6f,%.6e\n", r.M, r.N, r.K, r.amode, r.cplx, r.prec, r.gz, t, r.flops);
  }
  if (dump) std::fclose(dump);
  if (reset) eng->prof_used = 0;
  return UMX_OK;
}

int umx_debug_keep(umx_engine* eng, int on) {
  if (!eng) return UMX_ERR_ARG;
  eng->dbg_on = on != 0;
  if (!on) eng->dbg.clear();
  return UMX_OK;
}

int umx_debug_fetch(umx_engine* eng, const char* name, void* host_buf, size_t capacity, size_t* nbytes_out) {
  if (!eng || !name) return UMX_ERR_ARG;
  const std::string nm(name);
  if (nm.rfind("weights:", 0) == 0 || nm.rfind("experts:", 0) == 0) {
    if (!eng->have_weights) return fail(eng, UMX_ERR_ARG, "umx_debug_fetch: load weights first");
    HIPCHK(eng, hipSetDevice(eng->dev));
    HIPCHK(eng, hipStreamSynchronize(eng->stream));
    const void* dptr = nullptr; size_t nb = 0;
    std::string table; float ms = 0.f;
    if (nm == "weights:w") { dptr = eng->d_w; nb = eng->n_w * sizeof(float); }
    else if (nm == "weights:dw") { dptr = eng->d_dw; nb = eng->n_dw * sizeof(float); }
    else if (nm == "weights:bw") { dptr = eng->d_bw; nb = eng->n_bw * sizeof(unsigned short); }
    else if (nm == "weights:table") {
      for (const auto& kv : eng->wt) table += kv.first + " " + std::to_string(kv.second.off) + " " + std::to_string(kv.second.count) + "\n";
      nb = table.size();
    } else if (nm == "experts:kernel_ms") {
      if (!eng->experts_merged) return fail(eng, UMX_ERR_ARG, "umx_debug_fetch: no expert merge has run");
      HIPCHK(eng, hipEventElapsedTime(&ms, eng->ev_m0, eng->ev_m1));
      nb = sizeof(float);
    } else return fail(eng, UMX_ERR_ARG, std::string("umx_debug_fetch: no buffer named ") + name);
    if (nbytes_out) *nbytes_out = nb;
    if (host_buf) {
      if (capacity < nb) return fail(eng, UMX_ERR_ARG, "umx_debug_fetch: buffer too small");
      if (dptr) HIPCHK(eng, hipMemcpy(host_buf, dptr, nb, hipMemcpyDeviceToHost));
      else if (nm == "weights:table") std::memcpy(host_buf, table.data(), nb);
      else std::memcpy(host_buf, &ms, nb);
    }
    return UMX_OK;
  }
  auto it = eng->dbg.find(name);
  if (it == eng->dbg.end()) return fail(eng, UMX_ERR_ARG, std::string("umx_debug_fetch: no buffer named ") + name);
  if (nbytes_out) *nbytes_out = it->second.size();
  if (host_buf) {
    if (capacity < it->second.size()) return fail(eng, UMX_ERR_ARG, "umx_debug_fetch: buffer too small");
    std::memcpy(host_buf, it->second.data(), it->second.size());
  }
  return UMX_OK;
}

int umx_bond_changes(umx_engine* eng, int n, const double* r1, const double* r2, const double* cov, double bond_factor,
                     double margin_fraction, double delta_fraction, double* d1, double* d2, uint8_t* code) {
  if (!eng) return UMX_ERR_ARG;
  if (n <= 0 || !r1 || !r2 || !cov || !code) return fail(eng, UMX_ERR_ARG, "umx_bond_changes: bad arguments");
  if ((long)n * n > (1L << 31)) return fail(eng, UMX_ERR_CAPACITY, "umx_bond_changes: n*n exceeds 2^31 pairs");
  HIPCHK(eng, hipSetDevice(eng->dev));
  const size_t nn = (size_t)n * n, vb = (size_t)n * 3 * sizeof(double);
  double *d_r = nullptr, *d_d = nullptr; unsigned char* d_c = nullptr;
  HIPCHK(eng, hipMalloc(&d_r, 2 * vb + (size_t)n * sizeof(double)));
  hipError_t e1 = hipMalloc(&d_d, 2 * nn * sizeof(double)), e2 = hipMalloc(&d_c, nn);
  if (e1 != hipSuccess || e2 != hipSuccess) {
    (void)hipFree(d_r); if (d_d) (void)hipFree(d_d); if (d_c) (void)hipFree(d_c);
    return fail(eng, UMX_ERR_HIP, "umx_bond_changes: hipMalloc of the pair matrices failed");
  }
  double* d_r2 = d_r + (size_t)n * 3; double* d_cov = d_r2 + (size_t)n * 3;
  hipStream_t s = eng->stream;
  int st = UMX_OK;
  auto ok = [&](hipError_t e, const char* what) { if (e != hipSuccess && st == UMX_OK) st = fail(eng, UMX_ERR_HIP, std::string(what) + ": " + hipGetErrorName(e)); };
  ok(hipMemcpyAsync(d_r, r1, vb, hipMemcpyHostToDevice, s), "copy r1");
  ok(hipMemcpyAsync(d_r2, r2, vb, hipMemcpyHostToDevice, s), "copy r2");
  ok(hipMemcpyAsync(d_cov, cov, (size_t)n * sizeof(double), hipMemcpyHostToDevice, s), "copy cov");
  if (st == UMX_OK) {
    dim3 grid((n + 63) / 64, (n + 3) / 4);
    umx::k_bond_changes<<<grid, 256, 0, s>>>(d_r, d_r2, d_cov, n, bond_factor, margin_fraction, delta_fraction, d_d, d_d + nn, d_c);
    ok(hipGetLastError(), "k_bond_changes");
    if (d1) ok(hipMemcpyAsync(d1, d_d, nn * sizeof(double), hipMemcpyDeviceToHost, s), "copy d1");
    if (d2) ok(hipMemcpyAsync(d2, d_d + nn, nn * sizeof(double), hipMemcpyDeviceToHost, s), "copy d2");
    ok(hipMemcpyAsync(code, d_c, nn, hipMemcpyDeviceToHost, s), "copy code");
  }
  ok(hipStreamSynchronize(s), "sync");
  (void)hipFree(d_r); (void)hipFree(d_d); (void)hipFree(d_c);
  return st;
}

}
```

pdb2reaction_amd/csrc/umx_engine.h:

```cpp
#pragma once
#include <hip/hip_runtime.h>
#include <algorithm>
#include <cmath>
#include <cstdio>
#include <cstdlib>
#include <chrono>
#include <cstring>
#include <functional>
#include <initializer_list>
#include <map>
#include <memory>
#include <set>
#include <string>
#include <type_traits>
#include <vector>

#include "../../include/umx.h"
#include "umx_common.h"
#include "umx_gemm.h"
#include "umx_gemm_pl.h"
#include "umx_gemm_q.h"
#include "umx_kernels_pl.h"
#include "umx_kernels.h"
#include "umx_radial.h"
#include "umx_peer.h"

using namespace umx;

namespace {

std::string g_create_err;

struct Tensor { size_t off = 0; std::vector<int> shape; size_t count = 0; };

struct RadialW {
  const float *w1g, *w1gT, *ln1w, *ln1b, *w2, *w2T, *b2, *ln2w, *ln2b, *w3, *w3T, *b3;
  const double *tsd, *ttd;
  int out;
};
struct LayerW {
  const float *n1w, *n1b, *n2w, *n2b;
  const float *c1m0, *c1m0b, *c1m0T, *c1m1, *c1m1T, *c1m2, *c1m2T;
  const float *c2m0, *c2m0b, *c2m0T, *c2m1, *c2m1T, *c2m2, *c2m2T;
  const float *smlp, *smlpb, *smlpT, *l1w, *l1b, *l1T, *l2w, *l2b, *l2T;
  const float *g1w, *g1b, *g1T, *g2w, *g2b, *g2T, *g3w, *g3b, *g3T;
  RadialW rad;
};

struct PosPtr {
  const float* f = nullptr;
  const double* d = nullptr;
  PosPtr(const float* p) : f(p) {}
  PosPtr(const double* p) : d(p) {}
  PosPtr atom(long i) const { return d ? PosPtr(d + i * 3) : PosPtr(f + i * 3); }
};

struct ProfRec { hipEvent_t a, b; double flops; int M, N, K, amode, cplx, prec, gz; };

struct Precision {
  const char* name = "bf16x3";
  bool planes = true;
  int fwd_fmt = 3;
  int rev_planes = 3;
  bool fwd_f16() const { return planes && fwd_fmt == 1; }
  bool rev_quad() const { return planes && rev_planes == 3; }
  const char* range_hint() const {
    return fwd_f16() ? " (an activation beyond the fp16 operand range of the split-f16 forward planes: re-load with UMX_PRECISION=split-bf16, bf16x3 or fp32)"
                     : " (non-finite input or an overflow in float32)";
  }
};

bool resolve_precision(const std::string& mode, Precision* out) {
  Precision p;
  if (mode == "auto" || mode == "bf16x3" || mode == "split-exact") p = {"bf16x3", true, 3, 3};
  else if (mode == "split" || mode == "split-f16") p = {"split-f16", true, 1, 2};
  else if (mode == "split-bf16") p = {"split-bf16", true, 3, 2};
  else if (mode == "fp32") p = {"fp32", false, 3, 2};
  else return false;
  if (out) *out = p;
  return true;
}

enum Pass { FWD, REV };

struct PlaneCopy {
  const unsigned short* ptr;
  bool quad;
  float scale;
};

constexpr int MAX_EXPERTS = 64;
constexpr int N_EXPERT_W = 6 * NL;
struct ExpertAlpha { double a[MAX_EXPERTS]; };
struct PackScales { float s[N_EXPERT_W]; };
struct MergeJob {
  const float* stack;
  float* w;
  float* wT;
  int rows, cols, half;
  int blk0;
};
struct PackJob {
  const float* src;
  unsigned short* dst;
  int rows, K, P;
  int quad, alignw;
  int f16;
  int blk0;
};

struct WS {
  int *deg, *row_ptr, *stats;
  float* xs[2 * NL + 1];
  float* xn[NL];
  float *xn2, *ffhg, *xf, *pre1, *pre2, *enode;
  float* gspre[NL];
  float* ffh[NL];
  float* ffg1[NL];
  float* ffg2[NL];
  float *gridA, *gridB;
  float *G0, *G1, *G2, *ggs, *n128a, *n128b;
  int *esrc, *edst, *ez, *out_ptr, *out_cur, *out_edge;
  float *evec, *frame, *dedd, *dedd_rad, *tau, *tau2, *gvec;
  float* h1pre[NL + 1];
  float* h2pre[NL + 1];
  float *ra, *rad_deg;
  float* rad[NL];
  float* hg[NL];
  float* msg[NL];
  float *xrot, *hid, *gmsg, *ghg, *gy1, *grad, *e128a;
  unsigned short *y1pl, *hidpl, *a2pl, *gmsgpl, *ghgpl, *gradpl;
};

struct Seg { bool matrix; std::function<int()> fn; float* sync_buf = nullptr; size_t sync_count = 0; };
struct Plan {
  std::vector<Seg> segs;
  void stream(std::function<int()> f) { segs.push_back({false, std::move(f)}); }
  void matrix(std::function<int()> f) { segs.push_back({true, std::move(f)}); }
  void sync(float* buf, size_t count) { Seg sg{false, nullptr}; sg.sync_buf = buf; sg.sync_count = count; segs.push_back(std::move(sg)); }
  int run_to_sync(size_t& at, const Seg** stop) {
    *stop = nullptr;
    while (at < segs.size()) {
      Seg& sg = segs[at++];
      if (sg.sync_buf) { *stop = &sg; return UMX_OK; }
      const int st = sg.fn();
      if (st != UMX_OK) return st;
    }
    return UMX_OK;
  }
};

}

struct umx_engine {
  int dev = 0;
  hipStream_t stream = nullptr;
  hipEvent_t ev_done = nullptr;
  bool ran_on_caller = false;
  int* d_flags = nullptr;
  hipStream_t stream2 = nullptr;
  hipEvent_t ev_fork = nullptr, ev_join = nullptr;
  hipEvent_t ev_tok[2] = {nullptr, nullptr};
  Precision prec;
  std::string precision;
  int low_sep = 3;
  int gemm_half = 5;
  int align = 2;
  float odd_sign = -1.0f;
  bool node_ctx = false;
  bool node_f64_on = true;
  int n_lanes = 0;
  long lanes_auto_edges = 0;
  int stream_cap = 512;
  bool throttle = false;
  bool gp = false; long gp_lo = 0, gp_hi = 0;
  std::unique_ptr<Plan> gp_plan;
  std::unique_ptr<WS> gp_ws;
  size_t gp_at = 0;
  hipStream_t gp_stream = nullptr;
  std::string err;
  bool have_weights = false;
  float* d_w = nullptr;
  float* d_dw = nullptr;
  double* d_dtab = nullptr;
  unsigned short* d_bw = nullptr;
  std::map<const float*, PlaneCopy> planes;
  std::map<std::string, Tensor> wt;
  std::vector<float> h_w;
  size_t n_w = 0, n_dw = 0, n_bw = 0;
  int n_experts = 0;
  bool experts_merged = false;
  float* d_ex = nullptr;
  MergeJob* d_mjobs = nullptr; PackJob* d_pjobs = nullptr; unsigned* d_mx = nullptr;
  int n_mjobs = 0, n_pjobs = 0, merge_blocks = 0, pack_blocks = 0;
  std::vector<const float*> f16_keys;
  hipEvent_t ev_m0 = nullptr, ev_m1 = nullptr;
  bool need_merge() const { return n_experts > 0 && !experts_merged; }
  RadialW rdeg{};
  LayerW lw[NL]{};
  const float *emb_sphere = nullptr, *normw = nullptr, *normb = nullptr, *e0 = nullptr, *e0b = nullptr, *e0T = nullptr,
              *e2 = nullptr, *e2b = nullptr, *e2T = nullptr, *e4 = nullptr, *e4b = nullptr;
  double rmsd = 1.0;
  std::vector<double> elem_refs;
  bool ff_grid = false;
  int grid_G = 0;
  int ws_grid() const { return ff_grid ? grid_G : 0; }
  const float *to_grid = nullptr, *from_grid = nullptr;
  bool grid_f64 = true;
  int emb_type = 0;
  int n_datasets = 5;
  std::string variant;
  bool have_system = false;
  int natoms = 0;
  float cutoff = 6.0f;
  int max_neigh = 300;
  int* d_z = nullptr;
  double* d_sysemb = nullptr;
  double* d_gmu = nullptr;
  double gcoef = 0.0;
  double refsum = 0.0;
  size_t ws_limit = 0;
  size_t ws_cap_default = (size_t)160 << 30;
  char* arena = nullptr;
  size_t arena_bytes = 0;
  long cap_nodes = 0, cap_edges = 0;
  int* d_deg_all = nullptr; int* d_cand_all = nullptr; long deg_all_cap = 0;
  int* d_img_edges = nullptr; long img_edges_cap = 0;
  int force_parts = 0;
  int* d_part_deg = nullptr; float* d_part_f = nullptr; long part_cap = 0;
  int recompute = 0;
  bool rc_active = false;
  bool arena_rc = false;
  bool arena_keep = false;
  int last_recompute = 0;
  int last_parts = 0;
  int last_lanes = 1;
  int arena_allocs = 0;
  bool ws_eager = false;
  long ws_soft_edges = 320000;
  double t_first_eval = -1.0;
  int hint_applied = 0;
  int hint_images = 0;
  float* d_io_pos = nullptr; double* d_io_e = nullptr; float* d_io_f = nullptr; long io_cap = 0, io_img_cap = 0;
  double* d_io_pos64 = nullptr; long io64_cap = 0;
  double* d_vir_part = nullptr; long vir_cap = 0;
  double* d_vir_wp = nullptr;
  double* vir_out = nullptr; int vir_slabs = 0;
  double* d_io_w = nullptr; long io_w_cap = 0;
  int64_t last_edges = 0; int32_t last_maxdeg = 0;
  bool pbc_on = false;
  double cell[9] = {0, 0, 0, 0, 0, 0, 0, 0, 0}; int pbc[3] = {0, 0, 0};
  Lattice64 lat{};
  Periodic per{};
  float per_cutoff = 0.f;
  float4* d_shifts = nullptr;
  int n_cells = 0;
  std::vector<double> cells;
  std::vector<int> cell_shifts;
  Periodic* d_cells = nullptr; long cells_cap = 0;
  Lattice64* d_lats = nullptr;
  float4* d_shifts_pk = nullptr; long shifts_pk_cap = 0;
  float* d_wrap = nullptr; long wrap_cap = 0;
  double* d_wrap64 = nullptr; long wrap64_cap = 0;
  int last_shifts = 0;
  bool pin_on = false;
  long pin_edges = 0; int pin_maxdeg = 0;
  bool pin_pbc_on = false; int pin_pbc[3] = {0, 0, 0};
  std::vector<int> pin_deg;
  std::vector<long> pin_row;
  std::vector<unsigned> pin_codes;
  int *d_pin_src = nullptr, *d_pin_dst = nullptr;
  int* d_pin_tix = nullptr;
  int* d_pin_wrap = nullptr;
  int* d_pin_deg = nullptr; long pin_deg_imgs = 0;
  float4* d_pin_shifts = nullptr; long pin_shifts_cap = 0;
  bool may_truncate = true;
  bool prof_on = false;
  std::vector<ProfRec> prof;
  size_t prof_used = 0;
  bool dbg_on = false;
  std::map<std::string, std::vector<char>> dbg;
};

namespace {

#define HIPCHK(eng, expr)                                                                         \
  do {                                                                                            \
    hipError_t _e = (expr);                                                                       \
    if (_e != hipSuccess) {                                                                       \
      (eng)->err = std::string(#expr) + ": " + hipGetErrorName(_e) + " (" + hipGetErrorString(_e) + ")"; \
      return UMX_ERR_HIP;                                                                         \
    }                                                                                             \
  } while (0)

#define CHK(expr) do { int _s = (expr); if (_s != UMX_OK) return _s; } while (0)

int fail(umx_engine* e, int code, const std::string& msg) { e->err = msg; return code; }

inline unsigned nblk(long n, int per) { return (unsigned)((n + per - 1) / per); }

struct DevBuf {
  void** p; size_t bytes;
  template <class T> DevBuf(T*& ptr, size_t count) : p(reinterpret_cast<void**>(&ptr)), bytes(count * sizeof(T)) {}
};
template <class Cap>
int grow(umx_engine* eng, Cap& cap, Cap new_cap, std::initializer_list<hipStream_t> drain, std::initializer_list<DevBuf> bufs) {
  for (hipStream_t s : drain) HIPCHK(eng, hipStreamSynchronize(s));
  for (const DevBuf& b : bufs) if (*b.p) HIPCHK(eng, hipFree(*b.p));
  for (const DevBuf& b : bufs) *b.p = nullptr;
  cap = 0;
  for (const DevBuf& b : bufs) HIPCHK(eng, hipMalloc(b.p, b.bytes));
  cap = new_cap;
  return UMX_OK;
}
inline long grown_edges(long e) { return e + e / 50 + 1024; }
int grow_arena(umx_engine* eng, hipStream_t s, size_t bytes) {
  CHK(grow(eng, eng->arena_bytes, bytes, {s, eng->stream2}, {DevBuf(eng->arena, bytes)}));
  ++eng->arena_allocs;
  return UMX_OK;
}

bool dbg_wanted(const std::string& name) {
  const char* ev = std::getenv("UMX_DEBUG_ONLY");
  if (!ev || !*ev) return true;
  const std::string only(ev);
  for (size_t a = 0; a <= only.size();) {
    size_t b = only.find(',', a);
    if (b == std::string::npos) b = only.size();
    if (b > a && name.compare(0, b - a, only, a, b - a) == 0) return true;
    a = b + 1;
  }
  return false;
}

int dbg_capture(umx_engine* eng, const std::string& name, const void* dptr, size_t bytes) {
  if (!eng->dbg_on || !dbg_wanted(name)) return UMX_OK;
  std::vector<char>& v = eng->dbg[name];
  v.resize(bytes);
  HIPCHK(eng, hipStreamSynchronize(eng->stream));
  if (bytes) HIPCHK(eng, hipMemcpy(v.data(), dptr, bytes, hipMemcpyDeviceToHost));
  return UMX_OK;
}
#define DBG(name, ptr, count) CHK(dbg_capture(eng, name, ptr, (size_t)(count) * sizeof(*(ptr))))

}
```

pdb2reaction_amd/csrc/umx_gemm.h:

```cpp
#pragma once
#include "umx_common.h"

namespace umx {

enum AMode { A_PLAIN = 0, A_MODUL = 1, A_SILU = 3 };

struct GemmP {
  const float* A; long lda; int offA0, offA1;
  const float* R; long ldr; int offR;
  const float* B; long ldb; int bHalf;
  float* Cp; long ldc; int offC, offCi;
  const float* bias;
  const float* resid; long ldres; int offRes;
  float conj;
  long zA, zC, zRes;
  long zBl;
  int M, N, K;
};

typedef float f32x16 __attribute__((ext_vector_type(16)));

constexpr int G_BK = 32;
constexpr int G_LDK = 36;


template <int BMR, int BNC> __device__ __forceinline__ bool xcd_tile(int M, int N, int& mt, int& nt) {
  const int nN = (N + BNC - 1) / BNC;
  const int nM = (M + BMR - 1) / BMR;
  const int xcd = blockIdx.x & 7, slot = blockIdx.x >> 3;
  mt = (slot / nN) * 8 + xcd; nt = slot % nN;
  return mt < nM;
}

template <int... V> constexpr long kernel_tag() {
  static_assert(((V >= 0 && V < 8) && ...), "one octal digit per parameter");
  long t = 1;
  ((t = t * 8 + V), ...);
  return t;
}

template <int BR> __device__ __forceinline__ int cplx_half(int t) { return t / BR; }
template <int BR> __device__ __forceinline__ int cplx_idx(int t) { return t % BR; }
template <int CPLX, int NT, int E, int BR> __device__ __forceinline__ int frag_row0(int w, int t) {
  return CPLX ? (cplx_half<NT / 2>(t) * BR + w * (E * NT / 2) + cplx_idx<NT / 2>(t) * E) : (w * (E * NT) + t * E);
}

template <int NR> __device__ __forceinline__ constexpr int cd_row(int r) { return NR == 16 ? (r & 3) + 8 * (r >> 2) : r; }

template <class Acc, int NR = sizeof(Acc) / sizeof(float)>
__device__ __forceinline__ void fold_low(Acc& acc, const Acc& low) {
#pragma unroll
  for (int r = 0; r < NR; ++r) {
    float v = low[r];
    asm("" : "+v"(v));
    acc[r] += v;
  }
}

typedef __bf16 bf16x8_t __attribute__((ext_vector_type(8)));
typedef float f32x2_t __attribute__((ext_vector_type(2)));
typedef float f32x4q_t __attribute__((ext_vector_type(4)));
typedef __bf16 bf16x2_t __attribute__((ext_vector_type(2)));
typedef unsigned int u32x4q_t __attribute__((ext_vector_type(4)));

__device__ __forceinline__ float qf_align_magic(const f32x4q_t& lo, const f32x4q_t& hi) {
  float m = __builtin_fmaxf(__builtin_fmaxf(__builtin_fabsf(lo[0]), __builtin_fabsf(lo[1])), __builtin_fabsf(lo[2]));
  m = __builtin_fmaxf(__builtin_fmaxf(m, __builtin_fabsf(lo[3])), __builtin_fabsf(hi[0]));
  m = __builtin_fmaxf(__builtin_fmaxf(m, __builtin_fabsf(hi[1])), __builtin_fabsf(hi[2]));
  m = __builtin_fmaxf(m, __builtin_fabsf(hi[3]));
  const unsigned int cb = ((__builtin_bit_cast(unsigned int, m) & 0x7f800000u) + 0x05800000u) | 0x00400000u;
  return __builtin_bit_cast(float, cb);
}
__device__ __forceinline__ float qf_round_q(float x, float c) {
  float t = x + c;
  asm("" : "+v"(t));
  return t - c;
}
__device__ __forceinline__ void qf_split2(float x0, float x1, float q0, float q1, unsigned int& p0, unsigned int& p1, unsigned int& p2) {
  p0 = __builtin_bit_cast(unsigned int, __builtin_convertvector(f32x2_t{q0, q1}, bf16x2_t));
  const float r0 = x0 - __builtin_bit_cast(float, p0 << 16), r1 = x1 - __builtin_bit_cast(float, p0 & 0xffff0000u);
  p1 = __builtin_bit_cast(unsigned int, __builtin_convertvector(f32x2_t{r0, r1}, bf16x2_t));
  const float s0 = r0 - __builtin_bit_cast(float, p1 << 16), s1 = r1 - __builtin_bit_cast(float, p1 & 0xffff0000u);
  p2 = __builtin_bit_cast(unsigned int, __builtin_convertvector(f32x2_t{s0, s1}, bf16x2_t));
}
template <int AL> __device__ __forceinline__ void qf_split(const f32x4q_t& lo, const f32x4q_t& hi, bf16x8_t (&a)[3]) {
  unsigned int w[3][4];
  const float c = AL ? qf_align_magic(lo, hi) : 0.f;
  auto pair = [&](float x0, float x1, int i) {
    if (AL) qf_split2(x0, x1, qf_round_q(x0, c), qf_round_q(x1, c), w[0][i], w[1][i], w[2][i]);
    else qf_split2(x0, x1, x0, x1, w[0][i], w[1][i], w[2][i]);
  };
  pair(lo[0], lo[1], 0); pair(lo[2], lo[3], 1); pair(hi[0], hi[1], 2); pair(hi[2], hi[3], 3);
#pragma unroll
  for (int q = 0; q < 3; ++q) { const u32x4q_t v{w[q][0], w[q][1], w[q][2], w[q][3]}; a[q] = __builtin_bit_cast(bf16x8_t, v); }
}

template <int CPLX>
__device__ __forceinline__ void gemm_epilogue(const GemmP& p, f32x16 (&acc)[2][2], int mt, int nt, int wm, int wn, int l31, int h) {
  if (CPLX) {
    const int chan = nt * 64 + wn * 32 + l31;
    const long e0 = (long)mt * 64 + wm * 32 + 4 * h;
    const bool full = ((long)mt * 64 + 64 <= p.M) && (nt * 64 + 64 <= p.N);
    float* c = p.Cp + e0 * p.ldc + chan;
    if (full) {
#pragma unroll
      for (int r = 0; r < 16; ++r) {
        float* cr = c + (long)cd_row<16>(r) * p.ldc;
        cr[p.offC] = acc[0][0][r] - p.conj * acc[1][1][r];
        cr[p.offCi] = acc[1][0][r] + p.conj * acc[0][1][r];
      }
    } else if (chan < p.N) {
#pragma unroll
      for (int r = 0; r < 16; ++r) {
        const int dr = cd_row<16>(r);
        if (e0 + dr < p.M) {
          float* cr = c + (long)dr * p.ldc;
          cr[p.offC] = acc[0][0][r] - p.conj * acc[1][1][r];
          cr[p.offCi] = acc[1][0][r] + p.conj * acc[0][1][r];
        }
      }
    }
  } else {
    const long zoffC = (long)blockIdx.z * p.zC, zoffR = (long)blockIdx.z * p.zRes;
    const bool full = ((long)mt * 128 + 128 <= p.M);
#pragma unroll
    for (int i = 0; i < 2; ++i)
#pragma unroll
      for (int j = 0; j < 2; ++j) {
        const int col = nt * 128 + wn * 64 + j * 32 + l31;
        const long row0 = (long)mt * 128 + wm * 64 + i * 32 + 4 * h;
        float* c = p.Cp + row0 * p.ldc + p.offC + zoffC + col;
        if (full && col < p.N && !p.resid) {
#pragma unroll
          for (int r = 0; r < 16; ++r) c[(long)cd_row<16>(r) * p.ldc] = acc[i][j][r];
        } else if (col < p.N) {
#pragma unroll
          for (int r = 0; r < 16; ++r) {
            const long row = row0 + cd_row<16>(r);
            if (row < p.M) {
              float v = acc[i][j][r];
              if (p.resid) v += p.resid[row * p.ldres + p.offRes + zoffR + col];
              p.Cp[row * p.ldc + p.offC + zoffC + col] = v;
            }
          }
        }
      }
  }
}

template <int AMODE, int CPLX>
__global__ __launch_bounds__(256, 2) void umx_gemm_kernel(const GemmP p) {
  __shared__ __attribute__((aligned(16))) float lds[2][2][128][G_LDK];
  constexpr int BMR = CPLX ? 64 : 128;
  constexpr int BNC = CPLX ? 64 : 128;
  const int tid = threadIdx.x, lane = tid & 63, wave = tid >> 6;
  const int wm = wave >> 1, wn = wave & 1;
  const int l31 = lane & 31, h = lane >> 5;

  int mt, nt;
  if (!xcd_tile<BMR, BNC>(p.M, p.N, mt, nt)) return;
  const long zoffA = (long)blockIdx.z * p.zA;
  const float* Bz = p.B + (p.zBl ? (blockIdx.z == 0 ? 0 : blockIdx.z < 4 ? 1 : 2) * p.zBl : 0);

  const int k4 = (tid & 7) * 4;
  const int trow0 = tid >> 3;
  float4 ra[4], rb[4];

  auto gload = [&](int kt) {
    const int k0 = kt * G_BK + k4;
#pragma unroll
    for (int r = 0; r < 4; ++r) {
      const int trow = trow0 + 32 * r;
      long grow; int offA;
      if (CPLX) { grow = (long)mt * 64 + (trow & 63); offA = (trow >> 6) ? p.offA1 : p.offA0; }
      else      { grow = (long)mt * 128 + trow;       offA = p.offA0; }
      float4 v = make_float4(0.f, 0.f, 0.f, 0.f);
      if (grow < p.M) {
        v = *reinterpret_cast<const float4*>(p.A + grow * p.lda + offA + zoffA + k0);
        if (AMODE == A_MODUL) {
          const float4 m = *reinterpret_cast<const float4*>(p.R + grow * p.ldr + p.offR + k0);
          v.x *= m.x; v.y *= m.y; v.z *= m.z; v.w *= m.w;
        }
        if (AMODE == A_SILU) { v.x = silu_f(v.x); v.y = silu_f(v.y); v.z = silu_f(v.z); v.w = silu_f(v.w); }
      }
      ra[r] = v;
      int brow; bool ok;
      if (CPLX) { const int c = nt * 64 + (trow & 63); ok = c < p.N; brow = (trow >> 6) * p.bHalf + c; }
      else      { brow = nt * 128 + trow; ok = brow < p.N; }
      rb[r] = ok ? *reinterpret_cast<const float4*>(Bz + (long)brow * p.ldb + k0) : make_float4(0.f, 0.f, 0.f, 0.f);
    }
  };
  auto lstore = [&](int buf) {
#pragma unroll
    for (int r = 0; r < 4; ++r) {
      const int trow = trow0 + 32 * r;
      *reinterpret_cast<float4*>(&lds[buf][0][trow][k4]) = ra[r];
      *reinterpret_cast<float4*>(&lds[buf][1][trow][k4]) = rb[r];
    }
  };

  f32x16 acc[2][2];
#pragma unroll
  for (int j = 0; j < 2; ++j) {
    const int col = nt * 128 + wn * 64 + j * 32 + l31;
    const float b0 = (!CPLX && p.bias && col < p.N && (p.zBl == 0 || blockIdx.z == 0)) ? p.bias[col] : 0.f;
#pragma unroll
    for (int i = 0; i < 2; ++i)
#pragma unroll
      for (int r = 0; r < 16; ++r) acc[i][j][r] = b0;
  }

  int arow[2], brow_l[2];
#pragma unroll
  for (int t = 0; t < 2; ++t) {
    arow[t]   = CPLX ? (t * 64 + wm * 32 + l31) : (wm * 64 + t * 32 + l31);
    brow_l[t] = CPLX ? (t * 64 + wn * 32 + l31) : (wn * 64 + t * 32 + l31);
  }

  const int nk = p.K / G_BK;
  gload(0);
  lstore(0);
  __syncthreads();
  for (int kt = 0; kt < nk; ++kt) {
    const int buf = kt & 1;
    if (kt + 1 < nk) gload(kt + 1);
#pragma unroll
    for (int kc = 0; kc < 4; ++kc) {
      float4 a[2], b[2];
#pragma unroll
      for (int t = 0; t < 2; ++t) {
        a[t] = *reinterpret_cast<const float4*>(&lds[buf][0][arow[t]][kc * 8 + 4 * h]);
        b[t] = *reinterpret_cast<const float4*>(&lds[buf][1][brow_l[t]][kc * 8 + 4 * h]);
      }
#pragma unroll
      for (int i = 0; i < 2; ++i)
#pragma unroll
        for (int j = 0; j < 2; ++j) {
          acc[i][j] = __builtin_amdgcn_mfma_f32_32x32x2f32(a[i].x, b[j].x, acc[i][j], 0, 0, 0);
          acc[i][j] = __builtin_amdgcn_mfma_f32_32x32x2f32(a[i].y, b[j].y, acc[i][j], 0, 0, 0);
          acc[i][j] = __builtin_amdgcn_mfma_f32_32x32x2f32(a[i].z, b[j].z, acc[i][j], 0, 0, 0);
          acc[i][j] = __builtin_amdgcn_mfma_f32_32x32x2f32(a[i].w, b[j].w, acc[i][j], 0, 0, 0);
        }
    }
    if (kt + 1 < nk) lstore(buf ^ 1);
    __syncthreads();
  }

  gemm_epilogue<CPLX>(p, acc, mt, nt, wm, wn, l31, h);
}


typedef double f64x4 __attribute__((ext_vector_type(4)));

template <int AMODE>
__global__ __launch_bounds__(256) void k_gemm_f64acc(const GemmP p) {
  constexpr int LD = 34;
  __shared__ double As[64][LD];
  __shared__ double Bs[64][LD];
  const int tid = threadIdx.x, lane = tid & 63, wave = tid >> 6;
  const int wm = wave >> 1, wn = wave & 1, l15 = lane & 15, lk = lane >> 4;
  const int nN = (p.N + 63) / 64;
  const int mt = blockIdx.x / nN, nt = blockIdx.x % nN;
  const long zoffA = (long)blockIdx.z * p.zA;
  const float* Bz = p.B + (p.zBl ? (blockIdx.z == 0 ? 0 : blockIdx.z < 4 ? 1 : 2) * p.zBl : 0);
  f64x4 acc[2][2];
#pragma unroll
  for (int i = 0; i < 2; ++i)
#pragma unroll
    for (int j = 0; j < 2; ++j) acc[i][j] = f64x4{0.0, 0.0, 0.0, 0.0};
  float ra[8], rb[8];
  auto fetch = [&](int k0) {
#pragma unroll
    for (int i = 0; i < 8; ++i) {
      const int idx = tid + 256 * i, r = idx >> 5, kk = idx & 31;
      const long grow = (long)mt * 64 + r;
      ra[i] = grow < p.M ? p.A[grow * p.lda + p.offA0 + zoffA + k0 + kk] : 0.f;
      const int brow = nt * 64 + r;
      rb[i] = brow < p.N ? Bz[(long)brow * p.ldb + k0 + kk] : 0.f;
    }
  };
  fetch(0);
  for (int k0 = 0; k0 < p.K; k0 += 32) {
#pragma unroll
    for (int i = 0; i < 8; ++i) {
      const int idx = tid + 256 * i, r = idx >> 5, kk = idx & 31;
      As[r][kk] = (double)(AMODE == A_SILU ? silu_f(ra[i]) : ra[i]);
      Bs[r][kk] = (double)rb[i];
    }
    __syncthreads();
    if (k0 + 32 < p.K) fetch(k0 + 32);
#pragma unroll
    for (int ks = 0; ks < 8; ++ks) {
      double a[2], b[2];
#pragma unroll
      for (int t = 0; t < 2; ++t) {
        a[t] = As[wm * 32 + t * 16 + l15][ks * 4 + lk];
        b[t] = Bs[wn * 32 + t * 16 + l15][ks * 4 + lk];
      }
#pragma unroll
      for (int i = 0; i < 2; ++i)
#pragma unroll
        for (int j = 0; j < 2; ++j) acc[i][j] = __builtin_amdgcn_mfma_f64_16x16x4f64(a[i], b[j], acc[i][j], 0, 0, 0);
    }
    __syncthreads();
  }
  const long zoffC = (long)blockIdx.z * p.zC, zoffR = (long)blockIdx.z * p.zRes;
#pragma unroll
  for (int i = 0; i < 2; ++i)
#pragma unroll
    for (int j = 0; j < 2; ++j) {
      const int col = nt * 64 + wn * 32 + j * 16 + l15;
      if (col >= p.N) continue;
      const double bv = (p.bias && (p.zBl == 0 || blockIdx.z == 0)) ? (double)p.bias[col] : 0.0;
#pragma unroll
      for (int r = 0; r < 4; ++r) {
        const long row = (long)mt * 64 + wm * 32 + i * 16 + lk + 4 * r;
        if (row >= p.M) continue;
        double v = acc[i][j][r] + bv;
        if (p.resid) v += (double)p.resid[row * p.ldres + p.offRes + zoffR + col];
        p.Cp[row * p.ldc + p.offC + zoffC + col] = (float)v;
      }
    }
}

}
```

pdb2reaction_amd/csrc/umx_gemm_q.h:

```cpp
#pragma once
#include <type_traits>
#include "umx_gemm_pl.h"

namespace umx {

template <int P> __device__ __forceinline__ int q_row_off(int row) { return (row >> 2) * (128 * P) + (row & 3) * (32 * P); }
template <int P> __device__ __forceinline__ int q_swz(int g) { return P == 3 ? ((g >> 2) & 1) : ((g >> 1) & 3); }
typedef _Float16 f16x8_t __attribute__((ext_vector_type(8)));

template <int JA, int JBF, int BHALF_ROUND, int A_BYTES, long TAG, int RND = 8192, class BO = long>
__device__ __forceinline__ void q3_issue(const unsigned char* A, const unsigned char* B, unsigned char* sbase, const BO (&a_off)[JA],
                                         const BO (&b_off)[JBF + BHALF_ROUND], long kofs_a, long kofs_b, int piece, bool b_tail) {
  BO ao[JA];
#pragma unroll
  for (int j = 0; j < JA; ++j) {
    ao[j] = a_off[j];
    if constexpr (sizeof(BO) == 4) asm("" : "+v"(ao[j]));
  }
#pragma unroll
  for (int j = 0; j < JA; ++j)
    __builtin_amdgcn_global_load_lds((A + kofs_a) + ao[j], (__attribute__((address_space(3))) void*)(sbase + piece + j * RND), 16, 0, 0);
  BO bo[JBF + BHALF_ROUND];
#pragma unroll
  for (int j = 0; j < JBF + BHALF_ROUND; ++j) {
    bo[j] = b_off[j];
    if constexpr (sizeof(BO) == 4) asm("" : "+v"(bo[j]));
  }
#pragma unroll
  for (int j = 0; j < JBF; ++j)
    __builtin_amdgcn_global_load_lds((B + kofs_b) + bo[j], (__attribute__((address_space(3))) void*)(sbase + A_BYTES + piece + j * RND), 16, 0, 0);
  if constexpr (BHALF_ROUND != 0)
    if (b_tail)
      __builtin_amdgcn_global_load_lds((B + kofs_b) + bo[JBF], (__attribute__((address_space(3))) void*)(sbase + A_BYTES + piece + JBF * RND), 16, 0, 0);
}

__host__ __device__ constexpr bool q_use_product(int PA, int PB, int NPROD, int qa, int qb) {
  if (PA == 3 && PB == 3) return qa + qb < 3;
  if (PA == 2 && PB == 3) return NPROD == 5 ? (qa + qb < 3) : (qa + qb < 2 || (qa == 0 && qb == 2));
  return NPROD == 4 ? true : (qa + qb < 2);
}

template <int CPLX, int WIDE, int P = 3, int S = 2, int F16 = 0, int NPROD = (P == 3 ? 6 : 3), int PB = P, int AF = 0, int LS = 0, int AL = 0, int MW = 4>
__global__ __launch_bounds__(MW * 128, MW == 4 ? 1 : 2) void umx_gemm_q_kernel(const GemmPL p) {
  static_assert(!AL || AF, "AL: the float32-A kernels");
  static_assert(!LS || (P == 3 && PB == 3 && !F16 && NPROD == 6), "LS: the six-product bf16 form");
  static_assert(LS != 2 || !WIDE, "LS = 2 (second accumulator set): 256 x 128 tiles only");
  static_assert(MW == 4 || MW == 2, "waves along M: 4 (256-row tiles) or 2 (half-height tiles, two workgroups per CU)");
  static_assert(!AF || (P == 3 && PB == 3 && F16 == 0), "AF: the six-product bf16 form with A as float32");
  static_assert((P == 3 && PB == 3 && NPROD == 6) || (P == 2 && PB == 2 && (NPROD == 3 || NPROD == 4)) || (P == 2 && PB == 3 && (NPROD == 4 || NPROD == 5)), "plane products");
  constexpr int NT = MW * 128, RND = NT * 16;
  constexpr int BM = 64 * MW, BN = WIDE ? 256 : 128;
  constexpr int BMR = CPLX ? BM / 2 : BM, BNC = CPLX ? BN / 2 : BN;
  constexpr int BLK = AF ? 256 : 128 * P, CPB = AF ? 16 : 8 * P;
  constexpr int BLKB = 128 * PB, CPBB = 8 * PB;
  constexpr int A_BYTES = AF ? BM * 64 : BM * 32 * P, B_BYTES = BN * 32 * PB, STAGE = A_BYTES + B_BYTES;
  constexpr int TNW = WIDE ? 4 : 2;
  constexpr int JA = A_BYTES / RND;
  constexpr int JBF = B_BYTES / RND, BHR = (B_BYTES % RND) ? 1 : 0;
  static_assert(S * STAGE * (MW == 4 ? 1 : 2) <= 160 * 1024 && A_BYTES % RND == 0 && (B_BYTES % RND == 0 || B_BYTES % RND == RND / 2), "tile geometry");
  static_assert((P == 2 || P == 3) && (PB == 2 || PB == 3), "two or three planes");
  static_assert(S >= 2 && S <= 4, "ring depth");
  __shared__ __attribute__((aligned(1024))) unsigned char ring[S * STAGE];
  const int tid = threadIdx.x, lane = tid & 63, wave = tid >> 6;
  const int wm = wave >> 1, wn = wave & 1;
  const int l31 = lane & 31, h = lane >> 5;

  int mt, nt;
  if (!xcd_tile<BMR, BNC>(p.M, p.N, mt, nt)) return;

  const unsigned char* Ab = reinterpret_cast<const unsigned char*>(p.Apl);
  const unsigned char* Bb = reinterpret_cast<const unsigned char*>(p.Bpl);
  const long a_blocks = p.lda / (16 * P);
  const long b_blocks = p.K / 16;
  const long gA = ((long)p.M + 3) / 4;
  const int gN = p.N / 4;
  typedef typename std::conditional<MW == 4, long, unsigned int>::type BOff;
  BOff a_off[JA], b_off[JBF + BHR];
  const long a_tile = MW == 4 ? 0 : (long)mt * (BMR / 4) * a_blocks * BLK;
#pragma unroll
  for (int j = 0; j < JA; ++j) {
    const int c = tid + NT * j, g = c / CPB, s = c % CPB;
    long grp; int offA;
    if (CPLX) { grp = (long)mt * (BMR / 4) + cplx_idx<BMR / 4>(g); offA = cplx_half<BMR / 4>(g) ? p.offA1 : p.offA0; }
    else      { grp = (long)mt * (BM / 4) + g;                offA = p.offA0; }
    if (grp >= gA) grp = gA - 1;
    if (AF) a_off[j] = (BOff)((grp * a_blocks + offA / 16) * BLK - a_tile + (s >> 2) * 64 + (((s & 3) ^ (g & 3)) * 16));
    else    a_off[j] = (BOff)((grp * a_blocks + offA / 16) * BLK - a_tile + (s ^ q_swz<P>(g)) * 16);
  }
#pragma unroll
  for (int j = 0; j < JBF + BHR; ++j) {
    const int c = tid + NT * j, g = (c / CPBB) % (BN / 4), s = c % CPBB;
    long grp;
    if (CPLX) { int cg = nt * (BNC / 4) + cplx_idx<BNC / 4>(g); if (cg >= gN) cg = gN - 1; grp = (long)cplx_half<BNC / 4>(g) * (p.bHalf / 4) + cg; }
    else      { int cg = nt * (BN / 4) + g; if (cg >= gN) cg = gN - 1; grp = cg; }
    b_off[j] = (BOff)(grp * b_blocks * BLKB + (s ^ q_swz<PB>(g)) * 16);
  }
  const int piece = __builtin_amdgcn_readfirstlane(wave * 1024);
  const bool b_tail = __builtin_amdgcn_readfirstlane(wave < MW ? 1 : 0) != 0;

  const float cs = F16 ? p.cscale : 1.f;
  const float cso = p.odd_sign < 0.f ? -cs : cs;
  f32x16 acc[2][TNW];
  f32x16 low[LS == 2 ? 2 : 1][LS == 2 ? TNW : 1];
  if constexpr (LS == 2) {
#pragma unroll
    for (int i = 0; i < 2; ++i)
#pragma unroll
      for (int j = 0; j < TNW; ++j)
#pragma unroll
        for (int r = 0; r < 16; ++r) low[i][j][r] = 0.f;
  }
#pragma unroll
  for (int j = 0; j < TNW; ++j) {
    float b0 = 0.f;
    if (!CPLX) {
      const int col = nt * BN + wn * (32 * TNW) + j * 32 + l31;
      b0 = (p.bias && col < p.N) ? p.bias[col] / cs : 0.f;
    }
    const float b1 = p.odd_sign < 0.f ? -b0 : b0;
#pragma unroll
    for (int i = 0; i < 2; ++i)
#pragma unroll
      for (int r = 0; r < 16; ++r) acc[i][j][r] = (r & 1) ? b1 : b0;
  }

  int a_ad[2][P], b_ad[TNW][PB];
#pragma unroll
  for (int t = 0; t < 2; ++t) {
    const int row = frag_row0<CPLX, 2, 32, BMR>(wm, t) + l31;
#pragma unroll
    for (int q = 0; q < P; ++q)
      a_ad[t][q] = AF ? ((row >> 2) * 256 + (row & 3) * 64 + ((((h * 2 + (q & 1)) ^ ((row >> 2) & 3))) * 16))
                      : (q_row_off<P>(row) + ((q * 2 + h) ^ q_swz<P>(row >> 2)) * 16);
  }
#pragma unroll
  for (int t = 0; t < TNW; ++t) {
    const int row = frag_row0<CPLX, TNW, 32, BNC>(wn, t) + l31;
#pragma unroll
    for (int q = 0; q < PB; ++q) b_ad[t][q] = A_BYTES + q_row_off<PB>(row) + ((q * 2 + h) ^ q_swz<PB>(row >> 2)) * 16;
  }

  const int nk = p.K / 16;
  constexpr long TAG = kernel_tag<CPLX, WIDE, P, S, F16, NPROD, PB, AF, LS, AL, MW>();
  constexpr int GI = JA + JBF;
#pragma unroll
  for (int t = 0; t < S - 1; ++t)
    if (t < nk) q3_issue<JA, JBF, BHR, A_BYTES, TAG, RND, BOff>(Ab + a_tile, Bb, ring + t * STAGE, a_off, b_off, (long)t * BLK, (long)t * BLKB, piece, b_tail);
  int st_cur = 0, st_nxt = S - 1;
  for (int kt = 0; kt < nk; ++kt) {
    if (S == 2 || kt + S - 2 >= nk) wait_vmcnt<0>();
    else if (BHR != 0 && b_tail) wait_vmcnt<(S - 2) * (GI + 1)>();
    else wait_vmcnt<(S - 2) * GI>();
    __builtin_amdgcn_s_barrier();
    if (kt + S - 1 < nk) q3_issue<JA, JBF, BHR, A_BYTES, TAG, RND, BOff>(Ab + a_tile, Bb, ring + st_nxt * STAGE, a_off, b_off, (long)(kt + S - 1) * BLK, (long)(kt + S - 1) * BLKB, piece, b_tail);
    const unsigned char* sb = ring + st_cur * STAGE;
    st_cur = st_cur + 1 == S ? 0 : st_cur + 1;
    st_nxt = st_nxt + 1 == S ? 0 : st_nxt + 1;
    bf16x8_t a[2][P], b[TNW][PB];
    if constexpr (AF) {
#pragma unroll
      for (int t = 0; t < 2; ++t)
        qf_split<AL>(*reinterpret_cast<const f32x4q_t*>(sb + a_ad[t][0]), *reinterpret_cast<const f32x4q_t*>(sb + a_ad[t][1]), a[t]);
    } else {
#pragma unroll
      for (int q = 0; q < P; ++q)
#pragma unroll
        for (int t = 0; t < 2; ++t) a[t][q] = *reinterpret_cast<const bf16x8_t*>(sb + a_ad[t][q]);
    }
#pragma unroll
    for (int q = 0; q < PB; ++q)
#pragma unroll
      for (int t = 0; t < TNW; ++t) b[t][q] = *reinterpret_cast<const bf16x8_t*>(sb + b_ad[t][q]);
    if constexpr (LS == 1) {
#pragma unroll
      for (int i = 0; i < 2; ++i)
#pragma unroll
        for (int j = 0; j < TNW; ++j) {
          f32x16 lo = {0.f, 0.f, 0.f, 0.f, 0.f, 0.f, 0.f, 0.f, 0.f, 0.f, 0.f, 0.f, 0.f, 0.f, 0.f, 0.f};
          lo = __builtin_amdgcn_mfma_f32_32x32x16_bf16(a[i][2], b[j][0], lo, 0, 0, 0);
          lo = __builtin_amdgcn_mfma_f32_32x32x16_bf16(a[i][1], b[j][1], lo, 0, 0, 0);
          lo = __builtin_amdgcn_mfma_f32_32x32x16_bf16(a[i][0], b[j][2], lo, 0, 0, 0);
          acc[i][j] = __builtin_amdgcn_mfma_f32_32x32x16_bf16(a[i][1], b[j][0], acc[i][j], 0, 0, 0);
          acc[i][j] = __builtin_amdgcn_mfma_f32_32x32x16_bf16(a[i][0], b[j][1], acc[i][j], 0, 0, 0);
          acc[i][j] = __builtin_amdgcn_mfma_f32_32x32x16_bf16(a[i][0], b[j][0], acc[i][j], 0, 0, 0);
          fold_low(acc[i][j], lo);
        }
    } else if constexpr (F16 && P == 2 && PB == 3 && NPROD == 4) {
#pragma unroll
      for (int i = 0; i < 2; ++i)
#pragma unroll
        for (int j = 0; j < TNW; ++j) {
          f32x16 lo = {0.f, 0.f, 0.f, 0.f, 0.f, 0.f, 0.f, 0.f, 0.f, 0.f, 0.f, 0.f, 0.f, 0.f, 0.f, 0.f};
          lo = __builtin_amdgcn_mfma_f32_32x32x16_f16(__builtin_bit_cast(f16x8_t, a[i][0]), __builtin_bit_cast(f16x8_t, b[j][2]), lo, 0, 0, 0);
          lo = __builtin_amdgcn_mfma_f32_32x32x16_f16(__builtin_bit_cast(f16x8_t, a[i][0]), __builtin_bit_cast(f16x8_t, b[j][1]), lo, 0, 0, 0);
          lo = __builtin_amdgcn_mfma_f32_32x32x16_f16(__builtin_bit_cast(f16x8_t, a[i][1]), __builtin_bit_cast(f16x8_t, b[j][0]), lo, 0, 0, 0);
          acc[i][j] = __builtin_amdgcn_mfma_f32_32x32x16_f16(__builtin_bit_cast(f16x8_t, a[i][0]), __builtin_bit_cast(f16x8_t, b[j][0]), acc[i][j], 0, 0, 0);
          fold_low(acc[i][j], lo);
        }
    } else
#pragma unroll
    for (int ord = P + PB - 2; ord >= 0; --ord)
#pragma unroll
      for (int qa = 0; qa < P; ++qa) {
        const int qb = ord - qa;
        if (qb < 0 || qb >= PB || !q_use_product(P, PB, NPROD, qa, qb)) continue;
#pragma unroll
        for (int i = 0; i < 2; ++i)
#pragma unroll
          for (int j = 0; j < TNW; ++j) {
            if constexpr (F16) acc[i][j] = __builtin_amdgcn_mfma_f32_32x32x16_f16(__builtin_bit_cast(f16x8_t, a[i][qa]), __builtin_bit_cast(f16x8_t, b[j][qb]), acc[i][j], 0, 0, 0);
            else if constexpr (LS == 2) {
              if (qa + qb == 2) low[i][j] = __builtin_amdgcn_mfma_f32_32x32x16_bf16(a[i][qa], b[j][qb], low[i][j], 0, 0, 0);
              else acc[i][j] = __builtin_amdgcn_mfma_f32_32x32x16_bf16(a[i][qa], b[j][qb], acc[i][j], 0, 0, 0);
            } else acc[i][j] = __builtin_amdgcn_mfma_f32_32x32x16_bf16(a[i][qa], b[j][qb], acc[i][j], 0, 0, 0);
          }
      }
  }
  if constexpr (LS == 2) {
#pragma unroll
    for (int i = 0; i < 2; ++i)
#pragma unroll
      for (int j = 0; j < TNW; ++j) fold_low(acc[i][j], low[i][j]);
  }

  const bool full = ((long)mt * BMR + BMR <= p.M) && (nt * BNC + BNC <= p.N);
  if (CPLX) {
#pragma unroll
    for (int cg = 0; cg < TNW / 2; ++cg) {
      const int chan = nt * BNC + wn * (16 * TNW) + cg * 32 + l31;
      const long e0 = (long)mt * BMR + wm * 32 + 4 * h;
      float* c = p.Cp + e0 * p.ldc + chan;
      if (full) {
#pragma unroll
        for (int r = 0; r < 16; ++r) {
          float* cr = c + (long)cd_row<16>(r) * p.ldc;
          cr[p.offC] = ((r & 1) ? cso : cs) * (acc[0][cg][r] - p.conj * acc[1][TNW / 2 + cg][r]);
          cr[p.offCi] = ((r & 1) ? cso : cs) * (acc[1][cg][r] + p.conj * acc[0][TNW / 2 + cg][r]);
        }
      } else if (chan < p.N) {
#pragma unroll
        for (int r = 0; r < 16; ++r) {
          const int dr = cd_row<16>(r);
          if (e0 + dr < p.M) {
            float* cr = c + (long)dr * p.ldc;
            cr[p.offC] = ((r & 1) ? cso : cs) * (acc[0][cg][r] - p.conj * acc[1][TNW / 2 + cg][r]);
            cr[p.offCi] = ((r & 1) ? cso : cs) * (acc[1][cg][r] + p.conj * acc[0][TNW / 2 + cg][r]);
          }
        }
      }
    }
  } else {
#pragma unroll
    for (int i = 0; i < 2; ++i)
#pragma unroll
      for (int j = 0; j < TNW; ++j) {
        const int col = nt * BN + wn * (32 * TNW) + j * 32 + l31;
        const long row0 = (long)mt * BM + wm * 64 + i * 32 + 4 * h;
        float* c = p.Cp + row0 * p.ldc + p.offC + col;
        if (full) {
#pragma unroll
          for (int r = 0; r < 16; ++r) c[(long)cd_row<16>(r) * p.ldc] = ((r & 1) ? cso : cs) * acc[i][j][r];
        } else if (col < p.N) {
#pragma unroll
          for (int r = 0; r < 16; ++r) {
            const int dr = cd_row<16>(r);
            if (row0 + dr < p.M) c[(long)dr * p.ldc] = ((r & 1) ? cso : cs) * acc[i][j][r];
          }
        }
      }
  }
}

}
```

pdb2reaction_amd/csrc/umx_launch.h:

```cpp
#pragma once

namespace {

int prof_open(umx_engine* eng, ProfRec** out, double flops, int prec, long M, int N, int K, int amode = 0, int cplx = 0, int gz = 1) {
  *out = nullptr;
  if (!eng->prof_on) return UMX_OK;
  if (eng->prof_used == eng->prof.size()) {
    ProfRec r; HIPCHK(eng, hipEventCreate(&r.a)); HIPCHK(eng, hipEventCreate(&r.b)); r.flops = 0; eng->prof.push_back(r);
  }
  ProfRec* pr = &eng->prof[eng->prof_used++];
  pr->flops = flops; pr->M = (int)M; pr->N = N; pr->K = K; pr->amode = amode; pr->cplx = cplx; pr->gz = gz; pr->prec = prec;
  HIPCHK(eng, hipEventRecord(pr->a, eng->stream));
  *out = pr;
  return UMX_OK;
}
int prof_close(umx_engine* eng, ProfRec* pr) {
  if (pr) HIPCHK(eng, hipEventRecord(pr->b, eng->stream));
  return UMX_OK;
}
inline unsigned vgrid(const umx_engine* eng, unsigned blocks) {
  return (eng->throttle && eng->stream_cap > 0 && blocks > (unsigned)eng->stream_cap) ? (unsigned)eng->stream_cap : blocks;
}

inline void launch_scan(hipStream_t s, const int* deg, long n, int* row_ptr, int* stats) {
  hipLaunchKernelGGL(k_scan, dim3(1), dim3(1024), 0, s, deg, n, row_ptr, stats);
}

GemmP gp_zero() { GemmP p; std::memset(&p, 0, sizeof(p)); p.conj = 1.0f; return p; }

int launch_gemm(umx_engine* eng, const GemmP& p, int amode, int cplx, int gz = 1) {
  if (p.M <= 0) return UMX_OK;
  if (p.K % G_BK != 0) return fail(eng, UMX_ERR_ARG, "gemm: K not a multiple of 32");
  const int bmr = cplx ? 64 : 128, bnc = cplx ? 64 : 128;
  const long nM = (p.M + bmr - 1) / bmr, nN = (p.N + bnc - 1) / bnc;
  const long blocks = ((nM + 7) / 8) * 8 * nN;
  dim3 grid((unsigned)blocks, 1, (unsigned)gz), block(256);
  ProfRec* pr;
  CHK(prof_open(eng, &pr, cplx ? 8.0 * p.M * (double)p.N * p.K : 2.0 * p.M * (double)p.N * p.K * gz, 0, p.M, p.N, p.K, amode, cplx, gz));
  if (eng->node_f64_on && eng->node_ctx && !cplx && (amode == A_PLAIN || amode == A_SILU)) {
    const dim3 g64((unsigned)(((p.M + 63) / 64) * ((p.N + 63) / 64)), 1, (unsigned)gz);
    if (amode == A_SILU) hipLaunchKernelGGL(k_gemm_f64acc<A_SILU>, g64, block, 0, eng->stream, p);
    else hipLaunchKernelGGL(k_gemm_f64acc<A_PLAIN>, g64, block, 0, eng->stream, p);
    HIPCHK(eng, hipGetLastError());
    return prof_close(eng, pr);
  }
  switch (amode * 10 + cplx) {
    case A_PLAIN * 10 + 0: hipLaunchKernelGGL((umx_gemm_kernel<A_PLAIN, 0>), grid, block, 0, eng->stream, p); break;
    case A_PLAIN * 10 + 1: hipLaunchKernelGGL((umx_gemm_kernel<A_PLAIN, 1>), grid, block, 0, eng->stream, p); break;
    case A_MODUL * 10 + 0: hipLaunchKernelGGL((umx_gemm_kernel<A_MODUL, 0>), grid, block, 0, eng->stream, p); break;
    case A_MODUL * 10 + 1: hipLaunchKernelGGL((umx_gemm_kernel<A_MODUL, 1>), grid, block, 0, eng->stream, p); break;
    case A_SILU * 10 + 0: hipLaunchKernelGGL((umx_gemm_kernel<A_SILU, 0>), grid, block, 0, eng->stream, p); break;
    default: return fail(eng, UMX_ERR_ARG, "gemm: variant not instantiated");
  }
  HIPCHK(eng, hipGetLastError());
  return prof_close(eng, pr);
}

struct NodeCtx { umx_engine* e; explicit NodeCtx(umx_engine* eng) : e(eng) { e->node_ctx = true; } ~NodeCtx() { e->node_ctx = false; } };

int gemm_plain(umx_engine* eng, const float* A, long lda, int offA, const float* B, long ldb, const float* bias, float* Cp,
               long ldc, int offC, long M, int N, int K, int amode = A_PLAIN, int gz = 1, long zA = 0, long zC = 0,
               const float* resid = nullptr, long ldres = 0, int offRes = 0, long zRes = 0) {
  GemmP p = gp_zero();
  p.A = A; p.lda = lda; p.offA0 = offA; p.B = B; p.ldb = ldb; p.bias = bias; p.Cp = Cp; p.ldc = ldc; p.offC = offC;
  p.M = (int)M; p.N = N; p.K = K; p.zA = zA; p.zC = zC; p.resid = resid; p.ldres = ldres; p.offRes = offRes; p.zRes = zRes;
  return launch_gemm(eng, p, amode, 0, gz);
}

template <class... Args> int gemm_node(umx_engine* eng, Args... args) {
  NodeCtx node(eng);
  return gemm_plain(eng, args...);
}

template <class... Args> int gemm_grid(umx_engine* eng, Args... args) {
  if (!eng->grid_f64) return gemm_plain(eng, args...);
  NodeCtx node(eng);
  return gemm_plain(eng, args...);
}

int gemm_cplx(umx_engine* eng, const float* A, long lda, int offRe, int offIm, const float* R, long ldr, int offR, const float* B,
              long ldb, int bHalf, float* Cp, long ldc, int offCre, int offCim, long M, int N, int K, float conj) {
  GemmP p = gp_zero();
  p.A = A; p.lda = lda; p.offA0 = offRe; p.offA1 = offIm; p.R = R; p.ldr = ldr; p.offR = offR; p.B = B; p.ldb = ldb; p.bHalf = bHalf;
  p.Cp = Cp; p.ldc = ldc; p.offC = offCre; p.offCi = offCim; p.M = (int)M; p.N = N; p.K = K; p.conj = conj;
  return launch_gemm(eng, p, R ? A_MODUL : A_PLAIN, 1);
}

int so3_linear(umx_engine* eng, const float* A, const float* Wl, const float* bias, float* Cp, long nn, const float* resid) {
  GemmP p = gp_zero();
  p.A = A; p.lda = ROW; p.offA0 = 0; p.B = Wl; p.ldb = C; p.bias = bias; p.Cp = Cp; p.ldc = ROW; p.offC = 0;
  p.M = (int)nn; p.N = C; p.K = C; p.zA = C; p.zC = C; p.resid = resid; p.ldres = ROW; p.offRes = 0; p.zRes = C; p.zBl = (long)C * C;
  NodeCtx node(eng);
  return launch_gemm(eng, p, A_PLAIN, 0, S);
}

enum PlFamily { Q_F16, Q_BF16, PL3_ROWS, PL3, PL2_WIDE, PL2_M16, PL2_M32 };

struct PlKey {
  PlFamily fam = Q_F16; bool cplx = false, wide = false, ls = false, al = false, half = false;
  bool operator==(const PlKey& o) const { return fam == o.fam && cplx == o.cplx && wide == o.wide && ls == o.ls && al == o.al && half == o.half; }
};
struct PlKernel { PlKey key; void (*fn)(const GemmPL); };

#define UMX_Q(cplx, wide, ls, al, half) \
  {{Q_BF16, cplx != 0, wide != 0, ls != 0, al != 0, half != 0}, umx_gemm_q_kernel<cplx, wide, 3, 2, 0, 6, 3, 1, (ls ? (wide ? 1 : 2) : 0), al, (half ? 2 : 4)>}
#define UMX_Q4(cplx, wide, ls) UMX_Q(cplx, wide, ls, 0, 0), UMX_Q(cplx, wide, ls, 1, 0), UMX_Q(cplx, wide, ls, 0, 1), UMX_Q(cplx, wide, ls, 1, 1)
const PlKernel pl_kernels[] = {
    {{Q_F16, false, false}, umx_gemm_q_kernel<0, 0, 2, 2, 1, 4, 3>}, {{Q_F16, true, false}, umx_gemm_q_kernel<1, 0, 2, 2, 1, 4, 3>},
    {{Q_F16, false, true}, umx_gemm_q_kernel<0, 1, 2, 2, 1, 4, 3>},  {{Q_F16, true, true}, umx_gemm_q_kernel<1, 1, 2, 2, 1, 4, 3>},
    UMX_Q4(0, 0, 0), UMX_Q4(0, 0, 1), UMX_Q4(0, 1, 0), UMX_Q4(0, 1, 1),
    UMX_Q4(1, 0, 0), UMX_Q4(1, 1, 0), UMX_Q4(1, 1, 1),
    {{PL3_ROWS}, umx_gemm_pl_kernel<16, 0, 3, 2, 4, 2, 2, 2, 1>},
    {{PL3}, umx_gemm_pl_kernel<32, 0, 3, 2, 4, 2, 2, 2>},
    {{PL2_WIDE, false, true}, umx_gemm_pl_kernel<16, 0, 2, 2, 4, 2, 2, 4>}, {{PL2_WIDE, true, true}, umx_gemm_pl_kernel<16, 1, 2, 2, 4, 2, 2, 4>},
    {{PL2_M16, false}, umx_gemm_pl_kernel<16, 0, 2, 3, 4, 2, 2, 2>},        {{PL2_M16, true}, umx_gemm_pl_kernel<16, 1, 2, 3, 4, 2, 2, 2>},
    {{PL2_M32, false}, umx_gemm_pl_kernel<32, 0, 2, 3, 4, 2, 2, 2>},
};
#undef UMX_Q
#undef UMX_Q4

struct PlChoice { PlKey key; unsigned blocks = 0; long lda = 0, ldb = 0; int prec = 0; const char* err = nullptr; };
PlChoice choose_pl(const Precision& pm, Pass pass, bool w_quad, int cplx, long M, int N, int K, int a_cols, bool a_f32rows, int low_sep, int align, int half) {
  PlChoice c;
  c.key.cplx = cplx != 0;
  const bool fwd = pass == FWD;
  const int P = fwd ? 3 : pm.rev_planes;
  c.prec = (fwd && pm.fwd_fmt == 1) ? 24 : P;
  c.lda = (long)a_cols * P; c.ldb = (long)K * P;
  const int bmr = cplx ? 128 : 256;
  const long nM = (M + bmr - 1) / bmr;
  const bool fills = nM * (N / (cplx ? 128 : 256)) >= 256;
  c.key.ls = fwd && pm.fwd_fmt == 3 && (low_sep == 2 || (low_sep == 3 && !cplx) || (low_sep == 1 && !cplx && K == RH));
  c.key.wide = N % (cplx ? 128 : 256) == 0 && (fills || c.key.ls);
  int bnc = c.key.wide ? (cplx ? 128 : 256) : (cplx ? 64 : 128);
  if (fwd && pm.fwd_fmt == 1) {
    c.key.fam = Q_F16; c.lda = (long)a_cols * 2; c.ldb = (long)K * 3;
  } else if (fwd || (P == 3 && w_quad)) {
    c.key.fam = Q_BF16; c.lda = (long)a_cols * 3; c.ldb = (long)K * 3;
    c.key.al = fwd && (align == 1 || (align == 2 && !cplx));
  } else if (P == 3) {
    if (cplx || N > 128) { c.err = "gemm_pl: three-plane PL products are instantiated for the plain N <= 128 (radial fc3^T) products only"; return c; }
    c.key.fam = a_f32rows ? PL3_ROWS : PL3;
    if (a_f32rows) c.lda = (long)a_cols * 2;
  } else if (c.key.wide) {
    c.key.fam = PL2_WIDE;
  } else {
    c.key.fam = (cplx || K >= 512) ? PL2_M16 : PL2_M32;
  }
  c.key.half = c.key.fam == Q_BF16 && (half == 3 || (half == 4 && cplx) || (half == 5 && !c.key.ls && K >= 256) ||
                               (fwd && c.key.ls && (half == 2 || (half == 1 && !c.key.wide))));
  const long nMf = c.key.half ? (M + bmr / 2 - 1) / (bmr / 2) : nM;
  c.blocks = (unsigned)(((nMf + 7) / 8) * 8 * ((N + bnc - 1) / bnc));
  return c;
}

int gemm_pl(umx_engine* eng, int cplx, Pass pass, const unsigned short* Apl, int a_cols, int offA0, int offA1, const float* Wkey, int bHalf,
            const float* bias, float* Cp, long ldc, int offC, int offCi, long M, int N, int K, float conj, bool a_f32rows = false) {
  if (M <= 0) return UMX_OK;
  auto it = eng->planes.find(Wkey);
  if (it == eng->planes.end()) return fail(eng, UMX_ERR_ARG, "gemm_pl: weight has no PL copy");
  if (K % 32 != 0) return fail(eng, UMX_ERR_ARG, "gemm_pl: K not a multiple of 32");
  const PlaneCopy& w = it->second;
  const PlChoice c = choose_pl(eng->prec, pass, w.quad, cplx, M, N, K, a_cols, a_f32rows, eng->low_sep, eng->align, eng->gemm_half);
  if (c.err) return fail(eng, UMX_ERR_ARG, c.err);
  const PlKernel* k = nullptr;
  for (const PlKernel& e : pl_kernels)
    if (e.key == c.key) { k = &e; break; }
  if (!k) return fail(eng, UMX_ERR_ARG, "gemm_pl: variant not instantiated");
  GemmPL q;
  std::memset(&q, 0, sizeof(q));
  q.Apl = Apl; q.lda = c.lda; q.offA0 = offA0; q.offA1 = offA1; q.Bpl = w.ptr; q.ldb = c.ldb; q.bHalf = bHalf;
  q.Cp = Cp; q.ldc = ldc; q.offC = offC; q.offCi = offCi; q.bias = bias; q.conj = conj; q.M = (int)M; q.N = N; q.K = K;
  q.odd_sign = eng->odd_sign;
  if (c.key.fam == Q_F16) q.cscale = 1.0f / (QF16_SCALE * w.scale);
  ProfRec* pr;
  CHK(prof_open(eng, &pr, cplx ? 8.0 * M * (double)N * K : 2.0 * M * (double)N * K, c.prec, M, N, K, 9, cplx));
  hipLaunchKernelGGL(k->fn, dim3(c.blocks), dim3(c.key.half ? 256 : 512), 0, eng->stream, q);
  HIPCHK(eng, hipGetLastError());
  return prof_close(eng, pr);
}

struct So2Layout { int ld, m0, m1re, m1im, m1w, m2re, m2im, m2w; };
constexpr So2Layout SO2_Y1 = {XROT, 768, 768, 1280, 512, 1792, 2048, 256};
constexpr So2Layout SO2_HG = {HG, 640, 640, 896, 256, 1152, 1280, 128};
constexpr So2Layout SO2_MSG = {ROW, 384, 384, 640, 256, 896, 1024, 128};
constexpr int SO2_RAD_M1 = 768, SO2_RAD_M2 = 1280;

int so2_conv(umx_engine* eng, Pass pass, const void* A, const So2Layout& la, float* Cp, const So2Layout& lc, const float* Wm0, const float* Wm1,
             const float* Wm2, const float* bias, long ne, float conj, const float* R = nullptr) {
  if (eng->prec.planes) {
    const unsigned short* Apl = static_cast<const unsigned short*>(A);
    CHK(gemm_pl(eng, 0, pass, Apl, la.ld, 0, 0, Wm0, 0, bias, Cp, lc.ld, 0, 0, ne, lc.m0, la.m0, 1.0f));
    CHK(gemm_pl(eng, 1, pass, Apl, la.ld, la.m1re, la.m1im, Wm1, lc.m1w, nullptr, Cp, lc.ld, lc.m1re, lc.m1im, ne, lc.m1w, la.m1w, conj));
    return gemm_pl(eng, 1, pass, Apl, la.ld, la.m2re, la.m2im, Wm2, lc.m2w, nullptr, Cp, lc.ld, lc.m2re, lc.m2im, ne, lc.m2w, la.m2w, conj);
  }
  const float* Af = static_cast<const float*>(A);
  GemmP p = gp_zero();
  p.A = Af; p.lda = la.ld; p.R = R; p.ldr = R ? RAD : 0; p.B = Wm0; p.ldb = la.m0; p.bias = bias;
  p.Cp = Cp; p.ldc = lc.ld; p.M = (int)ne; p.N = lc.m0; p.K = la.m0;
  CHK(launch_gemm(eng, p, R ? A_MODUL : A_PLAIN, 0));
  CHK(gemm_cplx(eng, Af, la.ld, la.m1re, la.m1im, R, R ? RAD : 0, R ? SO2_RAD_M1 : 0, Wm1, la.m1w, lc.m1w, Cp, lc.ld, lc.m1re, lc.m1im, ne, lc.m1w, la.m1w, conj));
  return gemm_cplx(eng, Af, la.ld, la.m2re, la.m2im, R, R ? RAD : 0, R ? SO2_RAD_M2 : 0, Wm2, la.m2w, lc.m2w, Cp, lc.ld, lc.m2re, lc.m2im, ne, lc.m2w, la.m2w, conj);
}

}
```

Measured before the change: 1.949.

## Add 8-wave 128-row tile variant for low-separated real bf16 GEMMs

Adds an MT template parameter so each wave covers one 32-row MFMA tile instead of two. This gives 128-row tiles with 8 waves and two workgroups per CU for the real low-separated six-product bf16 GEMMs. In the LS=1 path, B fragments are loaded inside the inner loop to cut register pressure. A new engine setting (default 3) selects this variant for real forward LS products when the tile is wide or K>=256, and these cases take priority over the half-height variant. The aim is higher occupancy and lower register pressure, at the cost of less A/B reuse per wave and more launched blocks.

```diff
diff --git a/pdb2reaction_amd/csrc/gemm_bench.hip b/pdb2reaction_amd/csrc/gemm_bench.hip
--- a/pdb2reaction_amd/csrc/gemm_bench.hip
+++ b/pdb2reaction_amd/csrc/gemm_bench.hip
@@ -311,9 +311,14 @@
   for (long i = (long)blockIdx.x * blockDim.x + threadIdx.x; i < n; i += (long)gridDim.x * blockDim.x) d += a[i] != b[i];
   if (d) atomicAdd(out, d);
 }
-static int half_mode(long M) {
+static int half_mode(long M, bool ls32) {
   struct Shape { const char* name; int cplx, wide, N, K, a_cols, offA1, bHalf, ldc, offCi; void (*full)(const GemmPL); void (*half)(const GemmPL); };
-  const Shape shapes[] = {
+  const Shape shapes_ls32[] = {
+      {"conv-1 m0  plain 256x128 LS=2", 0, 0, 640, 768, 768, 0, 0, 640, 0, umx_gemm_q_kernel<0, 0, 3, 2, 0, 6, 3, 1, 2, 1>, umx_gemm_q_kernel<0, 0, 3, 2, 0, 6, 3, 1, 2, 1, 4, 1>},
+      {"conv-2 m0  plain 256x128 LS=2", 0, 0, 384, 384, 384, 0, 0, 384, 0, umx_gemm_q_kernel<0, 0, 3, 2, 0, 6, 3, 1, 2, 1>, umx_gemm_q_kernel<0, 0, 3, 2, 0, 6, 3, 1, 2, 1, 4, 1>},
+      {"fc3        plain 256x256 LS=1", 0, 1, 1536, 128, 128, 0, 0, 1536, 0, umx_gemm_q_kernel<0, 1, 3, 2, 0, 6, 3, 1, 1, 1>, umx_gemm_q_kernel<0, 1, 3, 2, 0, 6, 3, 1, 1, 1, 4, 1>},
+  };
+  const Shape shapes_half[] = {
       {"conv-1 m0  plain 256x128 LS=2", 0, 0, 640, 768, 768, 0, 0, 640, 0, umx_gemm_q_kernel<0, 0, 3, 2, 0, 6, 3, 1, 2, 1>, umx_gemm_q_kernel<0, 0, 3, 2, 0, 6, 3, 1, 2, 1, 2>},
       {"conv-2 m0  plain 256x128 LS=2", 0, 0, 384, 384, 384, 0, 0, 384, 0, umx_gemm_q_kernel<0, 0, 3, 2, 0, 6, 3, 1, 2, 1>, umx_gemm_q_kernel<0, 0, 3, 2, 0, 6, 3, 1, 2, 1, 2>},
       {"fc3        plain 256x256 LS=1", 0, 1, 1536, 128, 128, 0, 0, 1536, 0, umx_gemm_q_kernel<0, 1, 3, 2, 0, 6, 3, 1, 1, 1>, umx_gemm_q_kernel<0, 1, 3, 2, 0, 6, 3, 1, 1, 1, 2>},
@@ -322,7 +327,10 @@
   const long Mp = (M + 3) / 4 * 4;
   std::vector<float> h((size_t)1 << 22); for (auto& v : h) v = (rand() / (float)RAND_MAX) * 2 - 1;
   unsigned long long* d_nd; CK(hipMalloc(&d_nd, 8));
-  for (const Shape& sh : shapes) {
+  const Shape* shapes = ls32 ? shapes_ls32 : shapes_half;
+  const int nshapes = ls32 ? 3 : 4, alt_threads = ls32 ? 512 : 256;
+  for (int si = 0; si < nshapes; ++si) {
+    const Shape& sh = shapes[si];
     const int brows = sh.cplx ? 2 * sh.bHalf : sh.N;
     float *A, *B, *C0, *C1, *bias; unsigned char *Aqf, *Bq;
     const size_t an = (size_t)M * sh.a_cols, bn = (size_t)brows * sh.K, cn = (size_t)M * sh.ldc;
@@ -343,15 +351,15 @@
     GemmPL g0 = g, g1 = g; g0.Cp = C0; g1.Cp = C1;
     CK(hipMemset(C0, 0, cn * 4)); CK(hipMemset(C1, 0xff, cn * 4));
     const float t0 = timeit([&] { hipLaunchKernelGGL(sh.full, grid(256), dim3(512), 0, 0, g0); });
-    const float t1 = timeit([&] { hipLaunchKernelGGL(sh.half, grid(128), dim3(256), 0, 0, g1); });
+    const float t1 = timeit([&] { hipLaunchKernelGGL(sh.half, grid(128), dim3(alt_threads), 0, 0, g1); });
     const float t0b = timeit([&] { hipLaunchKernelGGL(sh.full, grid(256), dim3(512), 0, 0, g0); });
-    const float t1b = timeit([&] { hipLaunchKernelGGL(sh.half, grid(128), dim3(256), 0, 0, g1); });
+    const float t1b = timeit([&] { hipLaunchKernelGGL(sh.half, grid(128), dim3(alt_threads), 0, 0, g1); });
     CK(hipMemset(d_nd, 0, 8));
     hipLaunchKernelGGL(k_count_diff, dim3(4096), dim3(256), 0, 0, reinterpret_cast<const unsigned int*>(C0), reinterpret_cast<const unsigned int*>(C1), (long)cn, d_nd);
     unsigned long long nd = 0; CK(hipMemcpy(&nd, d_nd, 8, hipMemcpyDeviceToHost));
     const double fl = (sh.cplx ? 8.0 : 2.0) * M * sh.N * sh.K * 6;
-    printf("%-32s M %ld N %4d K %4d   256-row %7.3f / %7.3f ms (%6.0f TF/s executed)   128-row x2 %7.3f / %7.3f ms (%6.0f TF/s)   %+5.1f %%   differing output words %llu of %zu\n",
-           sh.name, M, sh.N, sh.K, t0, t0b, fl / std::min(t0, t0b) / 1e9, t1, t1b, fl / std::min(t1, t1b) / 1e9, 100.0 * (std::min(t1, t1b) / std::min(t0, t0b) - 1.0), nd, cn);
+    printf("%-32s M %ld N %4d K %4d   256-row %7.3f / %7.3f ms (%6.0f TF/s executed)   %s %7.3f / %7.3f ms (%6.0f TF/s)   %+5.1f %%   differing output words %llu of %zu\n",
+           sh.name, M, sh.N, sh.K, t0, t0b, fl / std::min(t0, t0b) / 1e9, ls32 ? "128-row 8 waves x2" : "128-row x2", t1, t1b, fl / std::min(t1, t1b) / 1e9, 100.0 * (std::min(t1, t1b) / std::min(t0, t0b) - 1.0), nd, cn);
     fflush(stdout);
     CK(hipFree(A)); CK(hipFree(B)); CK(hipFree(C0)); CK(hipFree(C1)); CK(hipFree(bias)); CK(hipFree(Aqf)); CK(hipFree(Bq));
   }
@@ -359,7 +367,7 @@
 }
 
 int main(int argc, char** argv) {
-  if (argc > 1 && !strcmp(argv[1], "half")) return half_mode(argc > 2 ? atol(argv[2]) : 1140000);
+  if (argc > 1 && (!strcmp(argv[1], "half") || !strcmp(argv[1], "ls32"))) return half_mode(argc > 2 ? atol(argv[2]) : 1140000, argv[1][0] == 'l');
   if (argc > 1 && !strcmp(argv[1], "f16")) return f16_mode(argc > 2 ? atol(argv[2]) : 569632, argc > 3 ? atoi(argv[3]) : 512, argc > 4 ? atoi(argv[4]) : 512);
   const long M = argc > 1 ? atol(argv[1]) : 569632; const int N = argc > 2 ? atoi(argv[2]) : 640, K = argc > 3 ? atoi(argv[3]) : 768;
   const long lda = 2304;
diff --git a/pdb2reaction_amd/csrc/umx_api.hip b/pdb2reaction_amd/csrc/umx_api.hip
--- a/pdb2reaction_amd/csrc/umx_api.hip
+++ b/pdb2reaction_amd/csrc/umx_api.hip
@@ -190,6 +190,7 @@
   if (const char* ev = std::getenv("UMX_ALT_ROWS")) e->odd_sign = std::atoi(ev) != 0 ? -1.0f : 1.0f;
   if (const char* ev = std::getenv("UMX_LOW_SEP")) e->low_sep = std::atoi(ev);
   if (const char* ev = std::getenv("UMX_GEMM_HALF")) e->gemm_half = std::atoi(ev);
+  if (const char* ev = std::getenv("UMX_GEMM_LS32")) e->gemm_ls32 = std::atoi(ev);
   if (const char* ev = std::getenv("UMX_ALIGN_PLANES")) e->align = std::atoi(ev);
   int prio_lo = 0, prio_hi = 0;
   if (hipSetDevice(device_ordinal) != hipSuccess || hipDeviceGetStreamPriorityRange(&prio_lo, &prio_hi) != hipSuccess ||
diff --git a/pdb2reaction_amd/csrc/umx_engine.h b/pdb2reaction_amd/csrc/umx_engine.h
--- a/pdb2reaction_amd/csrc/umx_engine.h
+++ b/pdb2reaction_amd/csrc/umx_engine.h
@@ -164,6 +164,7 @@
   Precision prec;
   std::string precision;
   int low_sep = 3;
+  int gemm_ls32 = 3;
   int gemm_half = 5;
   int align = 2;
   float odd_sign = -1.0f;
diff --git a/pdb2reaction_amd/csrc/umx_gemm.h b/pdb2reaction_amd/csrc/umx_gemm.h
--- a/pdb2reaction_amd/csrc/umx_gemm.h
+++ b/pdb2reaction_amd/csrc/umx_gemm.h
@@ -42,7 +42,8 @@
 template <int BR> __device__ __forceinline__ int cplx_half(int t) { return t / BR; }
 template <int BR> __device__ __forceinline__ int cplx_idx(int t) { return t % BR; }
 template <int CPLX, int NT, int E, int BR> __device__ __forceinline__ int frag_row0(int w, int t) {
-  return CPLX ? (cplx_half<NT / 2>(t) * BR + w * (E * NT / 2) + cplx_idx<NT / 2>(t) * E) : (w * (E * NT) + t * E);
+  if constexpr (CPLX) return cplx_half<NT / 2>(t) * BR + w * (E * NT / 2) + cplx_idx<NT / 2>(t) * E;
+  else return w * (E * NT) + t * E;
 }
 
 template <int NR> __device__ __forceinline__ constexpr int cd_row(int r) { return NR == 16 ? (r & 3) + 8 * (r >> 2) : r; }
diff --git a/pdb2reaction_amd/csrc/umx_gemm_q.h b/pdb2reaction_amd/csrc/umx_gemm_q.h
--- a/pdb2reaction_amd/csrc/umx_gemm_q.h
+++ b/pdb2reaction_amd/csrc/umx_gemm_q.h
@@ -40,24 +40,26 @@
   return NPROD == 4 ? true : (qa + qb < 2);
 }
 
-template <int CPLX, int WIDE, int P = 3, int S = 2, int F16 = 0, int NPROD = (P == 3 ? 6 : 3), int PB = P, int AF = 0, int LS = 0, int AL = 0, int MW = 4>
-__global__ __launch_bounds__(MW * 128, MW == 4 ? 1 : 2) void umx_gemm_q_kernel(const GemmPL p) {
+template <int CPLX, int WIDE, int P = 3, int S = 2, int F16 = 0, int NPROD = (P == 3 ? 6 : 3), int PB = P, int AF = 0, int LS = 0, int AL = 0, int MW = 4, int MT = 2>
+__global__ __launch_bounds__(MW * 128, (MW == 4 && MT == 2) ? 1 : 2) void umx_gemm_q_kernel(const GemmPL p) {
   static_assert(!AL || AF, "AL: the float32-A kernels");
   static_assert(!LS || (P == 3 && PB == 3 && !F16 && NPROD == 6), "LS: the six-product bf16 form");
   static_assert(LS != 2 || !WIDE, "LS = 2 (second accumulator set): 256 x 128 tiles only");
   static_assert(MW == 4 || MW == 2, "waves along M: 4 (256-row tiles) or 2 (half-height tiles, two workgroups per CU)");
+  static_assert(MT == 2 || (MT == 1 && MW == 4 && !CPLX), "32-row MFMA tiles per wave along M: 2, or 1 (real products, 8 waves, 128-row tiles)");
   static_assert(!AF || (P == 3 && PB == 3 && F16 == 0), "AF: the six-product bf16 form with A as float32");
   static_assert((P == 3 && PB == 3 && NPROD == 6) || (P == 2 && PB == 2 && (NPROD == 3 || NPROD == 4)) || (P == 2 && PB == 3 && (NPROD == 4 || NPROD == 5)), "plane products");
   constexpr int NT = MW * 128, RND = NT * 16;
-  constexpr int BM = 64 * MW, BN = WIDE ? 256 : 128;
+  constexpr int BM = 32 * MT * MW, BN = WIDE ? 256 : 128;
   constexpr int BMR = CPLX ? BM / 2 : BM, BNC = CPLX ? BN / 2 : BN;
   constexpr int BLK = AF ? 256 : 128 * P, CPB = AF ? 16 : 8 * P;
   constexpr int BLKB = 128 * PB, CPBB = 8 * PB;
   constexpr int A_BYTES = AF ? BM * 64 : BM * 32 * P, B_BYTES = BN * 32 * PB, STAGE = A_BYTES + B_BYTES;
   constexpr int TNW = WIDE ? 4 : 2;
+  constexpr bool TWO = MW == 2 || MT == 1;
   constexpr int JA = A_BYTES / RND;
   constexpr int JBF = B_BYTES / RND, BHR = (B_BYTES % RND) ? 1 : 0;
-  static_assert(S * STAGE * (MW == 4 ? 1 : 2) <= 160 * 1024 && A_BYTES % RND == 0 && (B_BYTES % RND == 0 || B_BYTES % RND == RND / 2), "tile geometry");
+  static_assert(S * STAGE * (TWO ? 2 : 1) <= 160 * 1024 && A_BYTES % RND == 0 && (B_BYTES % RND == 0 || B_BYTES % RND == RND / 2), "tile geometry");
   static_assert((P == 2 || P == 3) && (PB == 2 || PB == 3), "two or three planes");
   static_assert(S >= 2 && S <= 4, "ring depth");
   __shared__ __attribute__((aligned(1024))) unsigned char ring[S * STAGE];
@@ -74,9 +76,9 @@
   const long b_blocks = p.K / 16;
   const long gA = ((long)p.M + 3) / 4;
   const int gN = p.N / 4;
-  typedef typename std::conditional<MW == 4, long, unsigned int>::type BOff;
+  typedef typename std::conditional<!TWO, long, unsigned int>::type BOff;
   BOff a_off[JA], b_off[JBF + BHR];
-  const long a_tile = MW == 4 ? 0 : (long)mt * (BMR / 4) * a_blocks * BLK;
+  const long a_tile = !TWO ? 0 : (long)mt * (BMR / 4) * a_blocks * BLK;
 #pragma unroll
   for (int j = 0; j < JA; ++j) {
     const int c = tid + NT * j, g = c / CPB, s = c % CPB;
@@ -96,15 +98,15 @@
     b_off[j] = (BOff)(grp * b_blocks * BLKB + (s ^ q_swz<PB>(g)) * 16);
   }
   const int piece = __builtin_amdgcn_readfirstlane(wave * 1024);
-  const bool b_tail = __builtin_amdgcn_readfirstlane(wave < MW ? 1 : 0) != 0;
+  const bool b_tail = __builtin_amdgcn_readfirstlane(wave < NT / 128 ? 1 : 0) != 0;
 
   const float cs = F16 ? p.cscale : 1.f;
   const float cso = p.odd_sign < 0.f ? -cs : cs;
-  f32x16 acc[2][TNW];
-  f32x16 low[LS == 2 ? 2 : 1][LS == 2 ? TNW : 1];
+  f32x16 acc[MT][TNW];
+  f32x16 low[LS == 2 ? MT : 1][LS == 2 ? TNW : 1];
   if constexpr (LS == 2) {
 #pragma unroll
-    for (int i = 0; i < 2; ++i)
+    for (int i = 0; i < MT; ++i)
 #pragma unroll
       for (int j = 0; j < TNW; ++j)
 #pragma unroll
@@ -119,15 +121,15 @@
     }
     const float b1 = p.odd_sign < 0.f ? -b0 : b0;
 #pragma unroll
-    for (int i = 0; i < 2; ++i)
+    for (int i = 0; i < MT; ++i)
 #pragma unroll
       for (int r = 0; r < 16; ++r) acc[i][j][r] = (r & 1) ? b1 : b0;
   }
 
-  int a_ad[2][P], b_ad[TNW][PB];
-#pragma unroll
-  for (int t = 0; t < 2; ++t) {
-    const int row = frag_row0<CPLX, 2, 32, BMR>(wm, t) + l31;
+  int a_ad[MT][P], b_ad[TNW][PB];
+#pragma unroll
+  for (int t = 0; t < MT; ++t) {
+    const int row = frag_row0<CPLX, MT, 32, BMR>(wm, t) + l31;
 #pragma unroll
     for (int q = 0; q < P; ++q)
       a_ad[t][q] = AF ? ((row >> 2) * 256 + (row & 3) * 64 + ((((h * 2 + (q & 1)) ^ ((row >> 2) & 3))) * 16))
@@ -141,7 +143,7 @@
   }
 
   const int nk = p.K / 16;
-  constexpr long TAG = kernel_tag<CPLX, WIDE, P, S, F16, NPROD, PB, AF, LS, AL, MW>();
+  constexpr long TAG = kernel_tag<CPLX, WIDE, P, S, F16, NPROD, PB, AF, LS, AL, MW, MT>();
   constexpr int GI = JA + JBF;
 #pragma unroll
   for (int t = 0; t < S - 1; ++t)
@@ -156,26 +158,32 @@
     const unsigned char* sb = ring + st_cur * STAGE;
     st_cur = st_cur + 1 == S ? 0 : st_cur + 1;
     st_nxt = st_nxt + 1 == S ? 0 : st_nxt + 1;
-    bf16x8_t a[2][P], b[TNW][PB];
+    bf16x8_t a[MT][P], b[TNW][PB];
     if constexpr (AF) {
 #pragma unroll
-      for (int t = 0; t < 2; ++t)
+      for (int t = 0; t < MT; ++t)
         qf_split<AL>(*reinterpret_cast<const f32x4q_t*>(sb + a_ad[t][0]), *reinterpret_cast<const f32x4q_t*>(sb + a_ad[t][1]), a[t]);
     } else {
 #pragma unroll
       for (int q = 0; q < P; ++q)
 #pragma unroll
-        for (int t = 0; t < 2; ++t) a[t][q] = *reinterpret_cast<const bf16x8_t*>(sb + a_ad[t][q]);
-    }
+        for (int t = 0; t < MT; ++t) a[t][q] = *reinterpret_cast<const bf16x8_t*>(sb + a_ad[t][q]);
+    }
+    if constexpr (!(LS == 1 && MT == 1)) {
 #pragma unroll
     for (int q = 0; q < PB; ++q)
 #pragma unroll
       for (int t = 0; t < TNW; ++t) b[t][q] = *reinterpret_cast<const bf16x8_t*>(sb + b_ad[t][q]);
+    }
     if constexpr (LS == 1) {
 #pragma unroll
-      for (int i = 0; i < 2; ++i)
+      for (int i = 0; i < MT; ++i)
 #pragma unroll
         for (int j = 0; j < TNW; ++j) {
+          if constexpr (MT == 1) {
+#pragma unroll
+            for (int q = 0; q < PB; ++q) b[j][q] = *reinterpret_cast<const bf16x8_t*>(sb + b_ad[j][q]);
+          }
           f32x16 lo = {0.f, 0.f, 0.f, 0.f, 0.f, 0.f, 0.f, 0.f, 0.f, 0.f, 0.f, 0.f, 0.f, 0.f, 0.f, 0.f};
           lo = __builtin_amdgcn_mfma_f32_32x32x16_bf16(a[i][2], b[j][0], lo, 0, 0, 0);
           lo = __builtin_amdgcn_mfma_f32_32x32x16_bf16(a[i][1], b[j][1], lo, 0, 0, 0);
@@ -187,7 +195,7 @@
         }
     } else if constexpr (F16 && P == 2 && PB == 3 && NPROD == 4) {
 #pragma unroll
-      for (int i = 0; i < 2; ++i)
+      for (int i = 0; i < MT; ++i)
 #pragma unroll
         for (int j = 0; j < TNW; ++j) {
           f32x16 lo = {0.f, 0.f, 0.f, 0.f, 0.f, 0.f, 0.f, 0.f, 0.f, 0.f, 0.f, 0.f, 0.f, 0.f, 0.f, 0.f};
@@ -205,7 +213,7 @@
         const int qb = ord - qa;
         if (qb < 0 || qb >= PB || !q_use_product(P, PB, NPROD, qa, qb)) continue;
 #pragma unroll
-        for (int i = 0; i < 2; ++i)
+        for (int i = 0; i < MT; ++i)
 #pragma unroll
           for (int j = 0; j < TNW; ++j) {
             if constexpr (F16) acc[i][j] = __builtin_amdgcn_mfma_f32_32x32x16_f16(__builtin_bit_cast(f16x8_t, a[i][qa]), __builtin_bit_cast(f16x8_t, b[j][qb]), acc[i][j], 0, 0, 0);
@@ -218,13 +226,13 @@
   }
   if constexpr (LS == 2) {
 #pragma unroll
-    for (int i = 0; i < 2; ++i)
+    for (int i = 0; i < MT; ++i)
 #pragma unroll
       for (int j = 0; j < TNW; ++j) fold_low(acc[i][j], low[i][j]);
   }
 
   const bool full = ((long)mt * BMR + BMR <= p.M) && (nt * BNC + BNC <= p.N);
-  if (CPLX) {
+  if constexpr (CPLX) {
 #pragma unroll
     for (int cg = 0; cg < TNW / 2; ++cg) {
       const int chan = nt * BNC + wn * (16 * TNW) + cg * 32 + l31;
@@ -251,11 +259,11 @@
     }
   } else {
 #pragma unroll
-    for (int i = 0; i < 2; ++i)
+    for (int i = 0; i < MT; ++i)
 #pragma unroll
       for (int j = 0; j < TNW; ++j) {
         const int col = nt * BN + wn * (32 * TNW) + j * 32 + l31;
-        const long row0 = (long)mt * BM + wm * 64 + i * 32 + 4 * h;
+        const long row0 = (long)mt * BM + wm * (32 * MT) + i * 32 + 4 * h;
         float* c = p.Cp + row0 * p.ldc + p.offC + col;
         if (full) {
 #pragma unroll
diff --git a/pdb2reaction_amd/csrc/umx_launch.h b/pdb2reaction_amd/csrc/umx_launch.h
--- a/pdb2reaction_amd/csrc/umx_launch.h
+++ b/pdb2reaction_amd/csrc/umx_launch.h
@@ -97,19 +97,25 @@
 enum PlFamily { Q_F16, Q_BF16, PL3_ROWS, PL3, PL2_WIDE, PL2_M16, PL2_M32 };
 
 struct PlKey {
-  PlFamily fam = Q_F16; bool cplx = false, wide = false, ls = false, al = false, half = false;
-  bool operator==(const PlKey& o) const { return fam == o.fam && cplx == o.cplx && wide == o.wide && ls == o.ls && al == o.al && half == o.half; }
+  PlFamily fam = Q_F16; bool cplx = false, wide = false, ls = false, al = false, half = false, ls32 = false;
+  constexpr bool operator==(const PlKey& o) const {
+    return fam == o.fam && cplx == o.cplx && wide == o.wide && ls == o.ls && al == o.al && half == o.half && ls32 == o.ls32;
+  }
 };
 struct PlKernel { PlKey key; void (*fn)(const GemmPL); };
 
 #define UMX_Q(cplx, wide, ls, al, half) \
   {{Q_BF16, cplx != 0, wide != 0, ls != 0, al != 0, half != 0}, umx_gemm_q_kernel<cplx, wide, 3, 2, 0, 6, 3, 1, (ls ? (wide ? 1 : 2) : 0), al, (half ? 2 : 4)>}
 #define UMX_Q4(cplx, wide, ls) UMX_Q(cplx, wide, ls, 0, 0), UMX_Q(cplx, wide, ls, 1, 0), UMX_Q(cplx, wide, ls, 0, 1), UMX_Q(cplx, wide, ls, 1, 1)
-const PlKernel pl_kernels[] = {
+constexpr PlKernel pl_kernels[] = {
     {{Q_F16, false, false}, umx_gemm_q_kernel<0, 0, 2, 2, 1, 4, 3>}, {{Q_F16, true, false}, umx_gemm_q_kernel<1, 0, 2, 2, 1, 4, 3>},
     {{Q_F16, false, true}, umx_gemm_q_kernel<0, 1, 2, 2, 1, 4, 3>},  {{Q_F16, true, true}, umx_gemm_q_kernel<1, 1, 2, 2, 1, 4, 3>},
     UMX_Q4(0, 0, 0), UMX_Q4(0, 0, 1), UMX_Q4(0, 1, 0), UMX_Q4(0, 1, 1),
     UMX_Q4(1, 0, 0), UMX_Q4(1, 1, 0), UMX_Q4(1, 1, 1),
+    {{Q_BF16, false, false, true, false, false, true}, umx_gemm_q_kernel<0, 0, 3, 2, 0, 6, 3, 1, 2, 0, 4, 1>},
+    {{Q_BF16, false, false, true, true, false, true}, umx_gemm_q_kernel<0, 0, 3, 2, 0, 6, 3, 1, 2, 1, 4, 1>},
+    {{Q_BF16, false, true, true, false, false, true}, umx_gemm_q_kernel<0, 1, 3, 2, 0, 6, 3, 1, 1, 0, 4, 1>},
+    {{Q_BF16, false, true, true, true, false, true}, umx_gemm_q_kernel<0, 1, 3, 2, 0, 6, 3, 1, 1, 1, 4, 1>},
     {{PL3_ROWS}, umx_gemm_pl_kernel<16, 0, 3, 2, 4, 2, 2, 2, 1>},
     {{PL3}, umx_gemm_pl_kernel<32, 0, 3, 2, 4, 2, 2, 2>},
     {{PL2_WIDE, false, true}, umx_gemm_pl_kernel<16, 0, 2, 2, 4, 2, 2, 4>}, {{PL2_WIDE, true, true}, umx_gemm_pl_kernel<16, 1, 2, 2, 4, 2, 2, 4>},
@@ -118,9 +124,17 @@
 };
 #undef UMX_Q
 #undef UMX_Q4
+constexpr bool pl_keys_distinct() {
+  constexpr int n = sizeof(pl_kernels) / sizeof(pl_kernels[0]);
+  for (int i = 0; i < n; ++i)
+    for (int j = i + 1; j < n; ++j)
+      if (pl_kernels[i].key == pl_kernels[j].key) return false;
+  return n == 43;
+}
+static_assert(pl_keys_distinct(), "pl_kernels: 43 instantiations, no key twice");
 
 struct PlChoice { PlKey key; unsigned blocks = 0; long lda = 0, ldb = 0; int prec = 0; const char* err = nullptr; };
-PlChoice choose_pl(const Precision& pm, Pass pass, bool w_quad, int cplx, long M, int N, int K, int a_cols, bool a_f32rows, int low_sep, int align, int half) {
+PlChoice choose_pl(const Precision& pm, Pass pass, bool w_quad, int cplx, long M, int N, int K, int a_cols, bool a_f32rows, int low_sep, int align, int half, int ls32) {
   PlChoice c;
   c.key.cplx = cplx != 0;
   const bool fwd = pass == FWD;
@@ -149,7 +163,10 @@
   }
   c.key.half = c.key.fam == Q_BF16 && (half == 3 || (half == 4 && cplx) || (half == 5 && !c.key.ls && K >= 256) ||
                                (fwd && c.key.ls && (half == 2 || (half == 1 && !c.key.wide))));
-  const long nMf = c.key.half ? (M + bmr / 2 - 1) / (bmr / 2) : nM;
+  c.key.ls32 = c.key.fam == Q_BF16 && fwd && c.key.ls && !cplx &&
+               (ls32 == 2 || (ls32 == 1 && !c.key.wide) || (ls32 == 3 && (c.key.wide || K >= 256)));
+  if (c.key.ls32) c.key.half = false;
+  const long nMf = (c.key.half || c.key.ls32) ? (M + bmr / 2 - 1) / (bmr / 2) : nM;
   c.blocks = (unsigned)(((nMf + 7) / 8) * 8 * ((N + bnc - 1) / bnc));
   return c;
 }
@@ -161,7 +178,7 @@
   if (it == eng->planes.end()) return fail(eng, UMX_ERR_ARG, "gemm_pl: weight has no PL copy");
   if (K % 32 != 0) return fail(eng, UMX_ERR_ARG, "gemm_pl: K not a multiple of 32");
   const PlaneCopy& w = it->second;
-  const PlChoice c = choose_pl(eng->prec, pass, w.quad, cplx, M, N, K, a_cols, a_f32rows, eng->low_sep, eng->align, eng->gemm_half);
+  const PlChoice c = choose_pl(eng->prec, pass, w.quad, cplx, M, N, K, a_cols, a_f32rows, eng->low_sep, eng->align, eng->gemm_half, eng->gemm_ls32);
   if (c.err) return fail(eng, UMX_ERR_ARG, c.err);
   const PlKernel* k = nullptr;
   for (const PlKernel& e : pl_kernels)
```

Result: no change. 1.949 (median of 2 runs) (-0.0%).
